# pagmerek/frave

Hardware: AMD Instinct MI355X
Metric: Mpixels/s encode (transform+quant) at 4096x4096 (higher is better)
Workload: dtype u8->i32

## Files before the change

### frave_amd/api.py

```python
import ctypes as C
import os
import subprocess

import numpy as np

_HERE = os.path.dirname(os.path.abspath(__file__))
_SO = os.environ.get("FRI_HIP_LIBRARY") or os.path.join(_HERE, "libfri_hip.so")
NONE = -(2 ** 31)

SYMBOLS = [
    "fri_hip_strerror", "fri_hip_version", "fri_hip_ctx_create", "fri_hip_ctx_destroy", "fri_hip_backend",
    "fri_hip_last_hip_error", "fri_hip_plan_create", "fri_hip_plan_destroy", "fri_hip_plan_num_cells",
    "fri_hip_plan_num_bfs_cells", "fri_hip_plan_num_interior_cells", "fri_hip_plan_coef_count", "fri_hip_plan_pixel_bytes",
    "fri_hip_plan_centers", "fri_hip_plan_valid_mask", "fri_hip_plan_num_some", "fri_hip_plan_neighbour_cells",
    "fri_hip_plan_neighbour_table", "fri_hip_plan_tiling", "fri_hip_plan_tile_table", "fri_hip_transform_quant", "fri_hip_transform_quant_dev",
    "fri_hip_transform_quant_batch_dev", "fri_hip_transform_quant_batch", "fri_hip_predict_histogram",
    "fri_hip_predict_histogram_dev", "fri_hip_fit_value_sums", "fri_hip_fit_value_sums_dev", "fri_hip_fit_width_sums",
    "fri_hip_fit_width_sums_dev", "fri_hip_inverse_transform", "fri_hip_inverse_transform_dev",
    "fri_hip_time_transform_quant_dev", "fri_hip_plan_read_trace", "fri_hip_plan_inverse_lists",
    "fri_hip_shard_size", "fri_hip_shard_image", "fri_hip_multi_create", "fri_hip_multi_destroy", "fri_hip_multi_num_devices",
    "fri_hip_multi_plan", "fri_hip_multi_transform_quant", "fri_hip_predict_histogram_batch_dev", "fri_hip_fit_value_sums_batch_dev",
    "fri_hip_fit_width_sums_batch_dev", "fri_hip_solve6", "fri_hip_fit_value_params", "fri_hip_fit_width_params", "fri_hip_encode_image",
    "fri_hip_encode_image_dev", "fri_hip_inverse_transform_batch_dev", "fri_hip_predict_image", "fri_hip_predict_image_dev",
    "fri_hip_fit_params_batch_dev", "fri_hip_encode_image_batch_dev", "fri_hip_fit_value_params_batch_dev", "fri_hip_fit_width_params_batch_dev",
    "fri_hip_plan_assume_forward_coefficients", "fri_hip_encode_image_batch", "fri_hip_multi_encode_image",
    "fri_hip_plan_set_stream_order", "fri_hip_symbol_stream_batch_dev", "fri_hip_encode_image_symbols", "fri_hip_encode_symbols_batch_dev",
    "fri_hip_plan_set_dequantiser", "fri_hip_plan_tune_forward", "fri_hip_time_transform_quant_streams_dev",
    "fri_hip_plan_set_colour_transform", "fri_hip_quality_matrix", "fri_hip_measure_distortion_dev", "fri_hip_search_quality",
    "fri_hip_search_quality_dev", "fri_hip_estimate_size_dev", "fri_hip_estimate_size", "fri_hip_search_quality_for_size",
    "fri_hip_search_quality_for_size_dev", "fri_hip_plan_predict_grid", "fri_hip_plan_pred_slots", "fri_hip_measure_ssim_dev", "fri_hip_measure_ssim", "fri_hip_search_quality_ssim",
    "fri_hip_search_quality_ssim_dev",
    "fri_hip_plan420_create", "fri_hip_plan420_destroy", "fri_hip_plan420_luma", "fri_hip_plan420_chroma", "fri_hip_split420_dev", "fri_hip_merge420_dev",
    "fri_hip_measure_distortion420_dev", "fri_hip_encode_image420_symbols", "fri_hip_decode_image420", "fri_hip_search_quality420", "fri_hip_search_quality420_dev",
    "fri_hip_search_quality_for_size420", "fri_hip_search_quality_for_size420_dev", "fri_hip_search_quality_ssim420", "fri_hip_search_quality_ssim420_dev",
    "fri_hip_plan_rgba_create", "fri_hip_plan_rgba_destroy", "fri_hip_plan_rgba_colour", "fri_hip_plan_rgba_alpha", "fri_hip_split_rgba_dev", "fri_hip_merge_rgba_dev",
    "fri_hip_encode_symbols_rgba_dev", "fri_hip_encode_image_rgba_symbols", "fri_hip_decode_image_rgba",
    "fri_hip_plan_owned_pixels", "fri_hip_tile_shape", "fri_hip_plan_tiled_create", "fri_hip_plan_tiled_destroy", "fri_hip_plan_tiled_tile", "fri_hip_plan_tiled_grid",
    "fri_hip_split_tiles_dev", "fri_hip_merge_tiles_dev", "fri_hip_encode_symbols_tiled_dev", "fri_hip_encode_image_tiled_symbols", "fri_hip_decode_image_tiled",
    "fri_hip_measure_distortion_tiled_dev", "fri_hip_estimate_size_tiled_dev", "fri_hip_estimate_size_tiled", "fri_hip_search_quality_tiled", "fri_hip_search_quality_tiled_dev",
    "fri_hip_search_quality_ssim_tiled", "fri_hip_search_quality_ssim_tiled_dev", "fri_hip_search_quality_for_size_tiled", "fri_hip_search_quality_for_size_tiled_dev",
    "fri_hip_rans_scratch_bytes", "fri_hip_rans_encode_planes_dev", "fri_hip_rans_time_planes_dev", "fri_hip_encode_image_tiled_coded",
    "fri_hip_plan_tiled_region", "fri_hip_merge_tiles_region_dev", "fri_hip_decode_region_tiled_dev", "fri_hip_decode_region_tiled",
    "fri_hip_plan_tiled_region_cover", "fri_hip_split_tiles_region_dev", "fri_hip_encode_symbols_region_tiled_dev", "fri_hip_encode_region_tiled_symbols",
    "fri_hip_tile_shape420", "fri_hip_plan_tiled420_create", "fri_hip_plan_tiled420_destroy", "fri_hip_plan_tiled420_luma", "fri_hip_plan_tiled420_chroma",
    "fri_hip_plan_tiled420_grid", "fri_hip_plan_tiled420_region", "fri_hip_plan_tiled420_buffer_tiles", "fri_hip_split_tiles420_dev", "fri_hip_merge_tiles420_dev",
    "fri_hip_merge_tiles420_region_dev", "fri_hip_encode_symbols_tiled420_dev", "fri_hip_encode_image_tiled420_symbols", "fri_hip_decode_image_tiled420",
    "fri_hip_decode_region_tiled420_dev", "fri_hip_decode_region_tiled420",
    "fri_hip_measure_distortion_tiled420_dev", "fri_hip_estimate_size_tiled420_dev", "fri_hip_estimate_size_tiled420", "fri_hip_search_quality_tiled420",
    "fri_hip_search_quality_tiled420_dev", "fri_hip_search_quality_ssim_tiled420", "fri_hip_search_quality_ssim_tiled420_dev", "fri_hip_search_quality_for_size_tiled420",
    "fri_hip_search_quality_for_size_tiled420_dev", "fri_hip_encode_image_tiled420_coded",
    "fri_hip_decode_scratch_bytes", "fri_hip_decode_planes_dev", "fri_hip_decode_time_planes_dev", "fri_hip_decode_image_tiled_coded", "fri_hip_decode_image_tiled420_coded",
    "fri_hip_plan_num_some_levels", "fri_hip_preview_size", "fri_hip_decode_planes_levels_dev", "fri_hip_preview_tiles_dev", "fri_hip_preview_image_tiled",
    "fri_hip_preview_image_tiled_coded",
    "fri_hip_plan_tiled_regions", "fri_hip_merge_tiles_regions_dev", "fri_hip_decode_regions_tiled_dev", "fri_hip_decode_regions_tiled",
    "fri_hip_decode_regions_tiled_coded",
    "fri_hip_plan_tiled_rgba_create", "fri_hip_plan_tiled_rgba_destroy", "fri_hip_plan_tiled_rgba_colour", "fri_hip_plan_tiled_rgba_alpha", "fri_hip_plan_tiled_rgba_grid",
    "fri_hip_plan_tiled_rgba_region", "fri_hip_plan_tiled_rgba_buffer_tiles", "fri_hip_split_tiles_rgba_dev", "fri_hip_merge_tiles_rgba_dev",
    "fri_hip_merge_tiles_rgba_region_dev", "fri_hip_encode_symbols_tiled_rgba_dev", "fri_hip_encode_image_tiled_rgba_symbols", "fri_hip_decode_image_tiled_rgba",
    "fri_hip_decode_region_tiled_rgba_dev", "fri_hip_decode_region_tiled_rgba",
]
DECODE_TRUNCATED, DECODE_BAD_MODEL, DECODE_BAD_SLOT = 1, 2, 4
RANS_EMPTY_OK = 1
RANS_TOO_SMALL, RANS_BAD_MODEL, RANS_ZERO_FREQ, RANS_BAD_BUCKET = 1, 2, 4, 8
TILED_ALLOW_HOLES = 1
ALPHA_KEEP, ALPHA_CLEAN = 0, 1
COLOUR_NONE, COLOUR_RCT, COLOUR_YCBCR = 0, 1, 3
DEQUANT_REFERENCE, DEQUANT_MULTIPLY, DEQUANT_MIDPOINT = 0, 1, 2


class FriHipError(RuntimeError):
    def __init__(self, code, where, detail=""):
        self.code = code
        msg = load_library().fri_hip_strerror(code).decode()
        super().__init__(f"{where}: {msg} ({code}){': ' + detail if detail else ''}")


def library_path():
    return _SO

# ... 59 lines not shown
    L.fri_hip_transform_quant_dev.argtypes = [vp, vp, vp, vp, vp]
    L.fri_hip_transform_quant_batch_dev.argtypes = [vp, u32, vp, sz, vp, vp, sz, vp]
    L.fri_hip_transform_quant_batch.argtypes = [vp, u32, vp, vp, vp]
    L.fri_hip_predict_histogram.argtypes = [vp, vp, u32, vp, vp, vp, vp, vp, vp]
    L.fri_hip_predict_histogram_dev.argtypes = [vp, vp, u32, vp, vp, vp, vp, vp, vp, vp]
    L.fri_hip_fit_value_sums.argtypes = [vp, vp, u32, vp]
    L.fri_hip_fit_value_sums_dev.argtypes = [vp, vp, u32, vp, vp]
    L.fri_hip_fit_width_sums.argtypes = [vp, vp, u32, vp, vp, vp, vp]
    L.fri_hip_fit_width_sums_dev.argtypes = [vp, vp, u32, vp, vp, vp, vp]
    L.fri_hip_inverse_transform.argtypes = [vp, vp, vp, vp]
    L.fri_hip_inverse_transform_dev.argtypes = [vp, vp, vp, vp, vp]
    L.fri_hip_plan_read_trace.argtypes = [vp, vp]
    L.fri_hip_plan_inverse_lists.argtypes = [vp, vp]
    L.fri_hip_plan_predict_grid.argtypes = [vp, vp]
    L.fri_hip_plan_pred_slots.argtypes = [vp, vp]
    L.fri_hip_time_transform_quant_dev.argtypes = [vp, u32, vp, sz, vp, vp, sz, u32, vp, C.POINTER(C.c_double)]
    L.fri_hip_time_transform_quant_streams_dev.argtypes = [vp, u32, vp, sz, vp, vp, sz, u32, u32, C.POINTER(C.c_double)]
    L.fri_hip_plan_tune_forward.argtypes = [vp, u32, C.c_char_p, sz]
    L.fri_hip_shard_size.restype, L.fri_hip_shard_size.argtypes = u32, [u32, u32, u32]
    L.fri_hip_shard_image.restype, L.fri_hip_shard_image.argtypes = u32, [u32, u32, u32]
    L.fri_hip_multi_create.argtypes = [vp, u32, u32, u32, u32, C.POINTER(vp)]
    L.fri_hip_multi_destroy.argtypes = [vp]
    L.fri_hip_multi_num_devices.restype, L.fri_hip_multi_num_devices.argtypes = u32, [vp]
    L.fri_hip_multi_plan.restype, L.fri_hip_multi_plan.argtypes = vp, [vp, u32]
    L.fri_hip_multi_transform_quant.argtypes = [vp, u32, vp, vp, vp]
    L.fri_hip_predict_histogram_batch_dev.argtypes = [vp, u32, vp, sz, vp, vp, vp, sz, vp, vp, vp]
    L.fri_hip_fit_value_sums_batch_dev.argtypes = [vp, u32, vp, sz, vp, vp]
    L.fri_hip_fit_width_sums_batch_dev.argtypes = [vp, u32, vp, sz, vp, vp, vp, vp]
    L.fri_hip_solve6.restype, L.fri_hip_solve6.argtypes = None, [vp, vp, vp]
    L.fri_hip_fit_value_params.restype, L.fri_hip_fit_value_params.argtypes = None, [vp, vp]
    L.fri_hip_fit_width_params.restype, L.fri_hip_fit_width_params.argtypes = None, [vp, vp, vp, vp]
    L.fri_hip_encode_image.argtypes = [vp, vp, vp, i32, vp, vp, vp, vp, vp, vp, vp]
    L.fri_hip_encode_image_dev.argtypes = [vp, vp, vp, i32, vp, vp, vp, vp, vp, vp, vp, vp]
    L.fri_hip_inverse_transform_batch_dev.argtypes = [vp, u32, vp, sz, vp, vp, sz, vp]
    L.fri_hip_predict_image.argtypes = [vp, vp, i32, vp, vp, vp, vp, vp, vp]
    L.fri_hip_predict_image_dev.argtypes = [vp, vp, i32, vp, vp, vp, vp, vp, vp, vp]
    L.fri_hip_fit_params_batch_dev.argtypes = [vp, u32, vp, sz, vp, vp, vp]
    L.fri_hip_plan_assume_forward_coefficients.argtypes = [vp, i32]
    L.fri_hip_plan_set_dequantiser.argtypes = [vp, i32]
    L.fri_hip_plan_set_colour_transform.argtypes = [vp, i32]
    L.fri_hip_quality_matrix.argtypes = [i32, vp]
    L.fri_hip_measure_distortion_dev.argtypes = [vp, vp, vp, vp, vp, vp]
    L.fri_hip_search_quality.argtypes = [vp, vp, C.c_double, vp, vp]
    L.fri_hip_search_quality_dev.argtypes = [vp, vp, C.c_double, vp, vp, vp]
    L.fri_hip_estimate_size_dev.argtypes = [vp, u32, vp, vp, vp, vp, vp]
    L.fri_hip_estimate_size.argtypes = [vp, vp, vp, vp]
    L.fri_hip_search_quality_for_size.argtypes = [vp, vp, C.c_uint64, vp, vp]
    L.fri_hip_search_quality_for_size_dev.argtypes = [vp, vp, C.c_uint64, vp, vp, vp]
    L.fri_hip_measure_ssim_dev.argtypes = [vp, u32, vp, vp, sz, vp, vp]
    L.fri_hip_measure_ssim.argtypes = [vp, vp, vp, vp]
    L.fri_hip_search_quality_ssim.argtypes = [vp, vp, C.c_double, vp, vp]
    L.fri_hip_search_quality_ssim_dev.argtypes = [vp, vp, C.c_double, vp, vp, vp]
    L.fri_hip_plan_set_stream_order.argtypes = [vp, vp, C.c_uint64]
    L.fri_hip_symbol_stream_batch_dev.argtypes = [vp, u32, vp, sz, vp, vp, sz, vp, sz, vp]
    L.fri_hip_encode_image_symbols.argtypes = [vp, vp, vp, i32, vp, vp, vp, vp, vp]
    L.fri_hip_encode_symbols_batch_dev.argtypes = [vp, u32, vp, sz, vp, i32, vp, vp, sz, vp, sz, vp, sz, vp, vp, vp, vp]
    L.fri_hip_encode_image_batch.argtypes = [vp, u32, vp, vp, i32, vp, vp, vp, vp, vp, vp]
    L.fri_hip_multi_encode_image.argtypes = [vp, u32, vp, vp, i32, vp, vp, vp, vp, vp, vp]
    L.fri_hip_fit_value_params_batch_dev.argtypes = [vp, u32, vp, vp, vp]
    L.fri_hip_fit_width_params_batch_dev.argtypes = [vp, u32, vp, vp, vp, vp]
    L.fri_hip_encode_image_batch_dev.argtypes = [vp, u32, vp, sz, vp, i32, vp, vp, sz, vp, vp, sz, vp, vp, vp, vp]
    L.fri_hip_plan420_create.argtypes = [vp, u32, u32, C.POINTER(vp)]
    L.fri_hip_plan420_destroy.argtypes = [vp]
    L.fri_hip_plan420_luma.restype, L.fri_hip_plan420_luma.argtypes = vp, [vp]
    L.fri_hip_plan420_chroma.restype, L.fri_hip_plan420_chroma.argtypes = vp, [vp]
    L.fri_hip_split420_dev.argtypes = [vp, vp, vp, vp, vp]
    L.fri_hip_merge420_dev.argtypes = [vp, vp, vp, vp, vp]
    L.fri_hip_measure_distortion420_dev.argtypes = [vp, vp, vp, vp, vp, vp]
    L.fri_hip_encode_image420_symbols.argtypes = [vp, vp, i32, vp, vp, vp, vp, vp]
    L.fri_hip_decode_image420.argtypes = [vp, vp, i32, vp]
    L.fri_hip_search_quality420.argtypes = [vp, vp, C.c_double, vp, vp]
    L.fri_hip_search_quality420_dev.argtypes = [vp, vp, C.c_double, vp, vp, vp]
    L.fri_hip_search_quality_for_size420.argtypes = [vp, vp, C.c_uint64, vp, vp]
    L.fri_hip_search_quality_for_size420_dev.argtypes = [vp, vp, C.c_uint64, vp, vp, vp]
    L.fri_hip_search_quality_ssim420.argtypes = [vp, vp, C.c_double, vp, vp]
    L.fri_hip_search_quality_ssim420_dev.argtypes = [vp, vp, C.c_double, vp, vp, vp]
    L.fri_hip_plan_rgba_create.argtypes = [vp, u32, u32, C.POINTER(vp)]
    L.fri_hip_plan_rgba_destroy.argtypes = [vp]
    L.fri_hip_plan_rgba_colour.restype, L.fri_hip_plan_rgba_colour.argtypes = vp, [vp]
    L.fri_hip_plan_rgba_alpha.restype, L.fri_hip_plan_rgba_alpha.argtypes = vp, [vp]
    L.fri_hip_split_rgba_dev.argtypes = [vp, vp, i32, vp, vp, vp]
    L.fri_hip_merge_rgba_dev.argtypes = [vp, vp, vp, vp, vp]
    L.fri_hip_encode_symbols_rgba_dev.argtypes = [vp, vp, i32, vp, i32, vp, vp, vp, vp, vp, vp]
    L.fri_hip_encode_image_rgba_symbols.argtypes = [vp, vp, i32, vp, vp, vp, vp, vp, vp]
    L.fri_hip_decode_image_rgba.argtypes = [vp, vp, vp, vp]
    L.fri_hip_plan_owned_pixels.restype, L.fri_hip_plan_owned_pixels.argtypes = C.c_uint64, [vp]
    L.fri_hip_tile_shape.argtypes = [u32, u32, u32, vp, vp]
    L.fri_hip_plan_tiled_create.argtypes = [vp, u32, u32, u32, u32, u32, u32, C.POINTER(vp)]
    L.fri_hip_plan_tiled_destroy.argtypes = [vp]
    L.fri_hip_plan_tiled_tile.restype, L.fri_hip_plan_tiled_tile.argtypes = vp, [vp]
    L.fri_hip_plan_tiled_grid.argtypes = [vp, vp]
    L.fri_hip_split_tiles_dev.argtypes = [vp, vp, vp, vp]
    L.fri_hip_merge_tiles_dev.argtypes = [vp, vp, vp, vp]
    L.fri_hip_encode_symbols_tiled_dev.argtypes = [vp, vp, vp, i32, vp, vp, vp, vp, vp, vp]
    L.fri_hip_encode_image_tiled_symbols.argtypes = [vp, vp, vp, vp, vp, vp, vp, vp]
    L.fri_hip_decode_image_tiled.argtypes = [vp, vp, vp, vp]
    L.fri_hip_plan_tiled_region.argtypes = [vp, u32, u32, u32, u32, vp]
    L.fri_hip_merge_tiles_region_dev.argtypes = [vp, vp, u32, u32, u32, u32, vp, vp]
    L.fri_hip_decode_region_tiled_dev.argtypes = [vp, vp, vp, u32, u32, u32, u32, vp, vp]
    L.fri_hip_decode_region_tiled.argtypes = [vp, vp, vp, u32, u32, u32, u32, vp]
    L.fri_hip_plan_tiled_regions.argtypes = [vp, u32, vp, vp, C.c_size_t, vp, vp, C.c_size_t]
    L.fri_hip_merge_tiles_regions_dev.argtypes = [vp, vp, u32, u32, vp, vp, vp]
    L.fri_hip_decode_regions_tiled_dev.argtypes = [vp, vp, vp, u32, vp, vp, vp]
    L.fri_hip_decode_regions_tiled.argtypes = [vp, vp, vp, u32, vp, vp]
    L.fri_hip_decode_regions_tiled_coded.argtypes = [vp, u32, vp, vp, C.c_size_t, vp, vp, vp, vp, vp, vp, vp, vp]
    L.fri_hip_plan_tiled_region_cover.argtypes = [vp, u32, u32, u32, u32, vp]
# ... 318 lines not shown


class Plan:

    def __init__(self, ctx, width, height, channels, _handle=None):
        self._h = None
        self.ctx = ctx
        self.width, self.height, self.channels = width, height, channels
        self.colour_transform = COLOUR_NONE
        self._owns = _handle is None
        if _handle is None:
            h = C.c_void_p()
            _check(load_library().fri_hip_plan_create(ctx._h if ctx else None, width, height, channels, C.byref(h)), "fri_hip_plan_create", ctx)
        else:
            h = C.c_void_p(_handle)
        self._h = h
        L = load_library()
        self.num_cells = L.fri_hip_plan_num_cells(h)
        self.num_bfs_cells = L.fri_hip_plan_num_bfs_cells(h)
        self.num_interior_cells = L.fri_hip_plan_num_interior_cells(h)
        self.coef_count = L.fri_hip_plan_coef_count(h)
        self.pixel_bytes = L.fri_hip_plan_pixel_bytes(h)
        self.num_some = L.fri_hip_plan_num_some(h)

    def close(self):
        if self._h:
            if self._owns:
                load_library().fri_hip_plan_destroy(self._h)
            self._h = None

    def __del__(self):
        try:
            self.close()
        except Exception:
            pass

    def num_some_levels(self, levels):
        out = C.c_uint64(0)
        _check(load_library().fri_hip_plan_num_some_levels(self._h, int(levels), C.byref(out)), "fri_hip_plan_num_some_levels", self.ctx)
        return int(out.value)

    def owned_pixels(self):
        return int(load_library().fri_hip_plan_owned_pixels(self._h))

    def set_stream_order(self, order=None):
        if order is None:
            from . import emit

            order = emit.stream_order(self.centers(), self.valid_mask())
        order = np.ascontiguousarray(order, np.uint32)
        _check(load_library().fri_hip_plan_set_stream_order(self._h, _p(order), order.size), "fri_hip_plan_set_stream_order", self.ctx)
        return order

    def symbol_stream_batch_dev(self, n_planes, d_coefs, coef_stride, d_bucket, d_prediction, out_stride, d_symbols, symbol_stride, stream=0):
        _check(load_library().fri_hip_symbol_stream_batch_dev(self._h, n_planes, d_coefs, coef_stride, d_bucket, d_prediction, out_stride, d_symbols, symbol_stride, stream),
               "fri_hip_symbol_stream_batch_dev", self.ctx)

    def encode_symbols_batch_dev(self, n_images, d_pixels, pixel_stride, qmatrix, fit, d_params, d_coefs, coef_stride, d_node_words, word_stride, d_symbols, symbol_stride,
                                 d_hist, d_oob, d_fit_range=0, stream=0):
        q = _q(qmatrix)
        _check(load_library().fri_hip_encode_symbols_batch_dev(self._h, n_images, d_pixels, pixel_stride, _p(q), 1 if fit else 0, d_params, d_coefs, coef_stride, d_node_words,
                                                               word_stride, d_symbols, symbol_stride, d_hist, d_oob, d_fit_range, stream), "fri_hip_encode_symbols_batch_dev", self.ctx)

    def set_dequantiser(self, multiply):
        mode = (1 if multiply else 0) if isinstance(multiply, bool) else int(multiply)
        _check(load_library().fri_hip_plan_set_dequantiser(self._h, mode), "fri_hip_plan_set_dequantiser")

    def measure_distortion_dev(self, d_coefs, d_reference_pixels, d_out, qmatrix=None, stream=0):
        q = _q(qmatrix)
        _check(load_library().fri_hip_measure_distortion_dev(self._h, d_coefs, _p(q), d_reference_pixels, d_out, stream), "fri_hip_measure_distortion_dev", self.ctx)

    def search_quality(self, pixels, target_db, stream=0):
        return _search(self, "fri_hip_search_quality", pixels, float(target_db), C.c_double, stream)

    def measure_ssim(self, a, b):
        pa, pb = np.ascontiguousarray(a, np.uint8), np.ascontiguousarray(b, np.uint8)
        assert pa.size == self.pixel_bytes and pb.size == self.pixel_bytes
        out = np.zeros(self.channels + 1, np.int64)
        _check(load_library().fri_hip_measure_ssim(self._h, _p(pa), _p(pb), _p(out)), "fri_hip_measure_ssim", self.ctx)
        return out

    def measure_ssim_dev(self, d_a, d_b, d_out, n_images=1, pixel_stride=0, stream=0):
        _check(load_library().fri_hip_measure_ssim_dev(self._h, n_images, d_a, d_b, pixel_stride, d_out, stream), "fri_hip_measure_ssim_dev", self.ctx)

    def search_quality_ssim(self, pixels, target, stream=0):
        return _search(self, "fri_hip_search_quality_ssim", pixels, float(target), C.c_double, stream)

    def estimate_size(self, hist, oob=None, stream=0, n_images=1, d_bytes=None, d_models=None):
        L = load_library()
        if isinstance(hist, int):
            assert d_bytes
            _check(L.fri_hip_estimate_size_dev(self._h, n_images, hist, oob or None, d_bytes, d_models or None, stream), "fri_hip_estimate_size_dev", self.ctx)
            return None
        h = np.ascontiguousarray(hist, np.uint32)
        assert h.size == self.channels * 10 * 1024
        o = None if oob is None else np.ascontiguousarray(oob, np.uint64)
        assert o is None or o.size == self.channels
        out = C.c_uint64(0)
        _check(L.fri_hip_estimate_size(self._h, _p(h), None if o is None else _p(o), C.byref(out)), "fri_hip_estimate_size", self.ctx)
        return out.value

    def search_quality_for_size(self, pixels, max_bytes, stream=0):
        return _search(self, "fri_hip_search_quality_for_size", pixels, int(max_bytes), C.c_uint64, stream)

    def set_colour_transform(self, mode):
        _check(load_library().fri_hip_plan_set_colour_transform(self._h, int(mode)), "fri_hip_plan_set_colour_transform")
# ... 875 lines not shown
```

### frave_amd/csrc/fri_hip.cpp

```cpp
#include "fri_hip_internal.hpp"

#include <atomic>
#include <cstdio>
#include <cstdlib>
#include <mutex>
#include <new>
#include <optional>
#include <thread>

#include "search_scaffold.hpp"
#include "solve6.hpp"

using namespace fri;
using namespace fri::host;

void PlanDelete::operator()(fri_hip_plan *p) const { delete p; }

struct fri_hip_multi {
    std::vector<fri_hip_ctx *> ctxs;
    std::vector<fri_hip_plan *> plans;
};

namespace {

template <typename T>
hipError_t upload(std::vector<DevMem<void>> &bufs, const std::vector<T> &v, const T *&out, size_t pad = 0) {
    auto &d = bufs.emplace_back();
    if (hipError_t e = hipMalloc(d.put(), std::max<size_t>(v.size() + pad, 1) * sizeof(T))) return e;
    if (pad)
        if (hipError_t e = hipMemset(static_cast<T *>(d.get()) + v.size(), 0, pad * sizeof(T))) return e;
    if (!v.empty())
        if (hipError_t e = hipMemcpy(d, v.data(), v.size() * sizeof(T), hipMemcpyHostToDevice)) return e;
    out = static_cast<const T *>(d.get());
    return hipSuccess;
}

std::vector<float> laplace_table() {
    static const float width[10] = {2.5f, 4.5f, 6.3f, 8.5f, 12.7f, 16.f, 20.f, 24.f, 28.f, 36.f};
    std::vector<float> t(10 * 1024);
    for (int b = 0; b < 10; b++)
        for (uint32_t j = 0; j < 1024; j++) {
            const float x = (float)((j & 1u) ? (int32_t)(j + 1) / -2 : (int32_t)(j / 2));
            t[b * 1024 + j] = std::exp(-std::fabs(x - 0.0f) / width[b]) / (2.0f * width[b]);
        }
    return t;
}

struct Knobs {
    int band_rows = 0, cells_per_tile = 0, cells_per_wg = 0, target_wgs = 0, tile_bytes = 0;
    int ranks = 0;
    std::optional<int> strided_shares;
    bool has_rank_weights = false;
    float rank_weight[4] = {0, 0, 0, 0};
    bool pins_forward = false;
    int batch_share_tiles = 0;
    std::optional<int> inv_shared, inv_strided_shares;
    int inv_band_rows = 0;
    int pred_blocks = 0, hist_blocks = 0, trace = 0, k3_scan = 0;
    int k1_ablate = 0, k2_ablate = 0, k3_ablate = 0, k4_ablate = 0;
    std::optional<int> k1_cached_stores, k1_batch_shares, k4_older_eighths;
};

Knobs read_knobs() {
    Knobs k;
    const char *on = std::getenv("FRI_HIP_TUNING");
    if (!on || on[0] != '1' || on[1] != 0) return k;
    auto env = [](const char *name) { return std::getenv(name); };
    auto pin = [&](const char *name) {
        const char *s = env(name);
        k.pins_forward |= s != nullptr;
        return s;
    };
    auto opt = [](const char *s) { return s ? std::optional<int>(std::atoi(s)) : std::nullopt; };
    auto num = [&](const char *s) { return opt(s).value_or(0); };
    k.band_rows = num(pin("FRI_HIP_BAND_ROWS")), k.cells_per_tile = num(pin("FRI_HIP_CELLS_PER_TILE")), k.cells_per_wg = num(pin("FRI_HIP_CELLS_PER_WG"));
    k.target_wgs = num(pin("FRI_HIP_TARGET_WGS")), k.tile_bytes = num(pin("FRI_HIP_TILE_BYTES")), k.ranks = std::min(num(pin("FRI_HIP_RANKS")), 4);
    k.strided_shares = opt(pin("FRI_HIP_STRIDED_SHARES"));
    if (const char *s = pin("FRI_HIP_RANK_WEIGHTS")) {
        float *w = k.rank_weight;
        k.has_rank_weights = std::sscanf(s, "%f,%f,%f,%f", &w[0], &w[1], &w[2], &w[3]) == 4;
    }
    k.batch_share_tiles = num(env("FRI_HIP_BATCH_SHARE_TILES"));
    k.inv_shared = opt(env("FRI_HIP_INV_SHARED")), k.inv_strided_shares = opt(env("FRI_HIP_INV_STRIDED_SHARES")), k.inv_band_rows = num(env("FRI_HIP_INV_BAND_ROWS"));
    k.pred_blocks = num(env("FRI_HIP_PRED_BLOCKS")), k.hist_blocks = num(env("FRI_HIP_HIST_BLOCKS")), k.trace = num(env("FRI_HIP_TRACE")), k.k3_scan = num(env("FRI_HIP_K3_SCAN"));
    k.k1_ablate = num(env("FRI_HIP_K1_ABLATE")), k.k2_ablate = num(env("FRI_HIP_K2_ABLATE")), k.k3_ablate = num(env("FRI_HIP_K3_ABLATE")), k.k4_ablate = num(env("FRI_HIP_K4_ABLATE"));
    k.k1_cached_stores = opt(env("FRI_HIP_K1_CACHED_STORES")), k.k1_batch_shares = opt(env("FRI_HIP_K1_BATCH_SHARES")), k.k4_older_eighths = opt(env("FRI_HIP_K4_OLDER_EIGHTHS"));
    return k;
}

int acquire_acc(fri_hip_plan *p, hipStream_t stream, uint32_t n_planes = 1) {
    fri_hip_ctx *c = p->ctx;
    HIP_TRY(c, hipSetDevice(c->device));
    if (p->acc_dirty) {
        HIP_TRY(c, hipDeviceSynchronize());
        for (auto &a : p->acc_slots) {
            if (a.pred_acc) HIP_TRY(c, hipMemset(a.pred_acc, 0, (size_t)a.planes * kPredAccWords * sizeof(uint32_t)));
            if (a.fit_acc) HIP_TRY(c, hipMemset(a.fit_acc, 0, (size_t)a.planes * kFitShards * kFitAccWords * sizeof(unsigned long long)));
        }
        HIP_TRY(c, hipDeviceSynchronize());
        p->acc_dirty = false;
    }
    int idx = -1;
    for (uint32_t i = 0; i < kPredAccRing && idx < 0; i++)
        if (p->acc_slots[i].used && p->acc_slots[i].stream == stream) idx = (int)i;
    for (uint32_t i = 0; i < kPredAccRing && idx < 0; i++)
        if (!p->acc_slots[i].used) {
            p->acc_slots[i].used = true;
            p->acc_slots[i].stream = stream;
            idx = (int)i;
        }
    if (idx < 0) {
        auto &v = p->acc_slots[p->acc_next];
        idx = (int)p->acc_next;
        p->acc_next = (p->acc_next + 1) % kPredAccRing;
        if (!v.handed_over) HIP_TRY(c, hipEventCreateWithFlags(v.handed_over.put(), hipEventDisableTiming));
        hipError_t e = hipEventRecord(v.handed_over, v.stream);
        if (e == hipSuccess) e = hipStreamWaitEvent(stream, v.handed_over, 0);
        if (e != hipSuccess) {
            (void)hipGetLastError();
            HIP_TRY(c, hipDeviceSynchronize());
        }
        v.stream = stream;
    }
    auto &a = p->acc_slots[idx];
    if (a.planes < n_planes) {
        const uint32_t planes = std::min<uint32_t>(65535u, std::max<uint32_t>({4u, n_planes, 2u * a.planes}));
        AccBufs n;
        const size_t pb = (size_t)planes * kPredAccWords * sizeof(uint32_t), fb = (size_t)planes * kFitShards * kFitAccWords * sizeof(unsigned long long);
        hipError_t e = hipMalloc((void **)n.pred_acc.put(), pb);
        if (e == hipSuccess) e = hipMalloc((void **)n.fit_acc.put(), fb);
        if (e == hipSuccess) e = hipMalloc((void **)n.sums_int.put(), (size_t)planes * 3 * 28 * sizeof(unsigned long long));
        if (e == hipSuccess) e = hipMalloc((void **)n.sums_dbl.put(), (size_t)planes * 18 * sizeof(double));
        if (e == hipSuccess) e = hipMalloc((void **)n.range.put(), (size_t)planes * sizeof(unsigned long long));
        if (e == hipSuccess) e = hipMalloc((void **)n.params.put(), (size_t)planes * sizeof(PredictParams));
        if (e == hipSuccess) e = hipMemsetAsync(n.pred_acc, 0, pb, stream);
        if (e == hipSuccess) e = hipMemsetAsync(n.fit_acc, 0, fb, stream);
        if (e != hipSuccess) return fail_hip(c, e, "accumulator allocation");
        std::swap(static_cast<AccBufs &>(a), n);
// ... 417 lines not shown
        build_inverse_lists(p->geo, kInvListsMaxBytes);
    }
    if (!ctx) {
        p->dev.n_pred_tiles = p->geo.n_pred_tiles;
        p->dev.pred_blocks = (uint32_t)std::max(k.pred_blocks, 0), p->dev.hist_blocks = (uint32_t)std::max(k.hist_blocks, 0);
        p->dev.k4_older_eighths = k.k4_older_eighths.value_or(0);
        *out = plan.release();
        return FRI_HIP_OK;
    }
    if (hipSetDevice(ctx->device) != hipSuccess) return FRI_HIP_ERR_HIP;
    const Geometry &g = p->geo, &gi = p->inv_geo();
    DevicePlan &d = p->dev;
    std::vector<uint16_t> tab(&st.nbr_table[0][0], &st.nbr_table[0][0] + kCell * 6);
    std::vector<uint32_t> gather_off((size_t)kCell * 4);
    std::vector<uint16_t> pair_pos(256), heap_of_pos(kCell);
    build_gather_tables(tab.data(), gather_off.data(), pair_pos.data(), heap_of_pos.data());
    std::vector<uint32_t> halo_list(1024);
    build_halo_list(tab.data(), pair_pos.data(), halo_list.data());
    build_lf_deltas(tab.data(), d.lf_delta);
    bool node0_gathered = false;
    for (int n = 2; n < kCell; n++)
        for (int i = 0; i < 6; i++) node0_gathered |= !(tab[(size_t)n * 6 + i] & 0x8000u) && (tab[(size_t)n * 6 + i] & 511u) == 0;
    if (halo_list[0] == 0xFFFFFFFFu || node0_gathered || pair_pos[0] != 0) {
        return FRI_HIP_ERR_INVALID_ARGUMENT;
    }
    auto &bufs = p->owned;
    hipError_t e;
    if ((e = upload_tiling(bufs, g, d, false)) || (e = upload(bufs, g.centers, d.centers)) || (e = upload(bufs, g.interior, d.interior)) || (e = upload(bufs, g.valid_mask, d.valid_mask)) ||
        (e = upload(bufs, g.nbr_cells, d.nbr_cells)) || (e = upload(bufs, g.pred_slots, d.pred_slots)) || (e = upload(bufs, tab, d.nbr_table)) ||
        (e = upload(bufs, gather_off, d.gather_off)) || (e = upload(bufs, pair_pos, d.pair_pos)) || (e = upload(bufs, heap_of_pos, d.heap_of_pos)) ||
        (e = upload(bufs, halo_list, d.halo_list)) || (e = upload(bufs, laplace_table(), p->laplace)))
        return fail_hip(ctx, e, "plan tables");
    if (!gi.inv_lists.empty()) {
        if ((e = upload(bufs, gi.inv_lists, d.inv_lists)) || (e = upload(bufs, gi.inv_quads, d.inv_quads, kInvListPad)) || (e = upload(bufs, gi.inv_dwords, d.inv_dwords, kInvListPad)) ||
            (e = upload(bufs, gi.inv_parts, d.inv_parts, kInvListPad)))
            return fail_hip(ctx, e, "inverse lists");
        d.inv_rect_bytes = gi.inv_rect_bytes;
    }
    d.F = (uint32_t)g.centers.size(), d.width = (int32_t)g.width, d.height = (int32_t)g.height, d.channels = (int32_t)g.channels, d.n_pred_tiles = g.n_pred_tiles;
    d.covers_image = g.n_valid_leaves == (uint64_t)g.width * g.height;
    d.inv_group = fwd.many_shares && g.wg_tiles.size() > 1 && (g.wg_tiles.size() - 1) % 1024 == 0 ? (int32_t)((g.wg_tiles.size() - 1) / 1024) : 1;
    d.inv_max_wg_tiles = d.inv_group > 1 ? 0 : d.max_wg_tiles, d.inv_max_wg_cells = d.inv_group > 1 ? 0 : d.max_wg_cells;
    for (size_t sh = 0; d.inv_group > 1 && sh + d.inv_group < g.wg_tiles.size(); sh += d.inv_group) {
        const Tile &first = g.tiles[g.wg_tiles[sh]], &last = g.tiles[g.wg_tiles[sh + d.inv_group] - 1];
        d.inv_max_wg_cells = std::max(d.inv_max_wg_cells, last.cell_begin + last.cell_count - first.cell_begin);
        d.inv_max_wg_tiles = std::max(d.inv_max_wg_tiles, g.wg_tiles[sh + d.inv_group] - g.wg_tiles[sh]);
    }
    d.pred_blocks = k.pred_blocks > 0 ? (uint32_t)k.pred_blocks : (uint32_t)ctx->cu_count;
    d.hist_blocks = k.hist_blocks > 0 ? (uint32_t)k.hist_blocks : 2u * (uint32_t)ctx->cu_count;
    d.k1_ablate = k.k1_ablate;
    if (k.k1_cached_stores) d.k1_cached_stores = *k.k1_cached_stores > 0 ? 1 : 0;
    if (k.k1_batch_shares) d.k1_batch_shares = *k.k1_batch_shares != 0;
    d.k2_ablate = k.k2_ablate;
    d.k3_ablate = k.k3_ablate;
    d.k3_scan = k.k3_scan > 0;
    d.k4_ablate = k.k4_ablate;
    if (k.k4_older_eighths) d.k4_older_eighths = *k.k4_older_eighths;
    if (hipMalloc(bufs.emplace_back().put(), (size_t)d.pred_blocks * kPredJunkWaves * kPredJunkBytes) != hipSuccess) return FRI_HIP_ERR_HIP;
    d.junk = static_cast<uint8_t *>(bufs.back().get());
    if (k.trace > 0) {
        const size_t bytes = (size_t)std::max<size_t>(d.n_wg, p->own_inverse_tiling ? gi.wg_tiles.size() : 0) * 16 * sizeof(unsigned long long);
        auto &t = bufs.emplace_back();
        if (hipMalloc(t.put(), bytes) != hipSuccess || hipMemset(t, 0, bytes) != hipSuccess) return FRI_HIP_ERR_HIP;
        d.trace = static_cast<unsigned long long *>(t.get());
    }
    if (hipEventCreate(p->ev_begin.put()) != hipSuccess || hipEventCreate(p->ev_end.put()) != hipSuccess) return FRI_HIP_ERR_HIP;
    p->dev_inv = d;
    if (p->own_inverse_tiling && (e = upload_tiling(bufs, gi, p->dev_inv, true))) return fail_hip(ctx, e, "inverse tiling");
    p->fwd_tunable = p->own_inverse_tiling && !fwd.many_shares && !d.trace && !k.pins_forward;
    if (p->fwd_tunable) adopt_cached_forward_tiling(p);
    *out = plan.release();
    return FRI_HIP_OK;
}

int fri_hip_plan_destroy(fri_hip_plan *p) {
    if (p && p->ctx) (void)hipSetDevice(p->ctx->device);
    delete p;
    return FRI_HIP_OK;
}

uint32_t fri_hip_plan_num_cells(const fri_hip_plan *p) { return p ? (uint32_t)p->geo.centers.size() : 0; }
uint32_t fri_hip_plan_num_bfs_cells(const fri_hip_plan *p) { return p ? p->geo.n_bfs_cells : 0; }
uint32_t fri_hip_plan_num_interior_cells(const fri_hip_plan *p) { return p ? p->geo.n_interior : 0; }
size_t fri_hip_plan_coef_count(const fri_hip_plan *p) { return p ? (size_t)p->geo.channels * p->geo.centers.size() * kCell : 0; }
size_t fri_hip_plan_pixel_bytes(const fri_hip_plan *p) { return p ? (size_t)p->geo.width * p->geo.height * p->geo.channels : 0; }
uint64_t fri_hip_plan_num_some(const fri_hip_plan *p) { return p ? p->geo.n_some : 0; }
int fri_hip_plan_num_some_levels(const fri_hip_plan *p, uint32_t levels, uint64_t *out) {
    if (!p || !out || levels > (uint32_t)kDepth) return FRI_HIP_ERR_INVALID_ARGUMENT;
    *out = num_some_levels(p->geo, levels);
    return FRI_HIP_OK;
}
int fri_hip_preview_size(uint32_t width, uint32_t height, uint32_t shift, uint32_t out[2]) {
    if (!width || !height || shift > 4 || !out) return FRI_HIP_ERR_INVALID_ARGUMENT;
    const uint32_t S = 1u << shift;
    out[0] = (uint32_t)(((uint64_t)width + S - 1) / S), out[1] = (uint32_t)(((uint64_t)height + S - 1) / S);
    return FRI_HIP_OK;
}
uint64_t fri_hip_plan_owned_pixels(const fri_hip_plan *p) { return p ? p->geo.n_valid_leaves : 0; }

int fri_hip_plan_assume_forward_coefficients(fri_hip_plan *p, int on) {
    if (!p) return FRI_HIP_ERR_INVALID_ARGUMENT;
    p->assume_forward = on != 0;
    return FRI_HIP_OK;
}

int fri_hip_plan_set_dequantiser(fri_hip_plan *p, int mode) {
// ... 379 lines not shown
}

void fri_hip_fit_width_params(const int64_t wtw[3][21], const double wtr[3][6], const uint64_t rows[3], float width_params[3][6]) {
    Solve6Work w;
    for (int g = 0; g < 3; g++) fit_width_group(reinterpret_cast<const long long *>(wtw[g]), wtr[g], rows[g], width_params[g], w);
}

class Coefs16Lease {
  public:
    Coefs16Lease(fri_hip_plan *p, hipStream_t s, size_t planes) : p_(p), s_(s) { rc = take(planes); }
    ~Coefs16Lease() {
        if (rc) return;
        p_->coefs16_stream = s_, p_->coefs16_used = true;
        if (hipEventRecord(p_->ev_coefs16, s_) != hipSuccess) {
            (void)hipGetLastError();
            (void)hipDeviceSynchronize();
            p_->coefs16_used = false;
        }
    }
    Coefs16Lease(const Coefs16Lease &) = delete;
    Coefs16Lease &operator=(const Coefs16Lease &) = delete;
    int rc;

  private:
    int take(size_t planes) {
        fri_hip_ctx *c = p_->ctx;
        if (int r = grow(c, p_->coefs16, planes * p_->geo.centers.size() * kCell)) return r;
        if (!p_->ev_coefs16) HIP_TRY(c, hipEventCreateWithFlags(p_->ev_coefs16.put(), hipEventDisableTiming));
        if (p_->coefs16_used && p_->coefs16_stream != s_) HIP_TRY(c, hipStreamWaitEvent(s_, p_->ev_coefs16, 0));
        return FRI_HIP_OK;
    }
    fri_hip_plan *p_;
    hipStream_t s_;
};

static int fit_chain(fri_hip_plan *p, const PredBatch &b, unsigned long long *d_range, hipStream_t s, float *host_params = nullptr, unsigned long long *host_range = nullptr,
                     int trust = kPredAnyInt32) {
    if (!b.params) return FRI_HIP_ERR_INVALID_ARGUMENT;
    const int slot = acquire_acc(p, s, b.n_planes);
    if (slot < 0) return slot;
    auto &k = p->acc_slots[slot];
    float *params = const_cast<float *>(reinterpret_cast<const float *>(b.params));
    const uint64_t F = p->geo.centers.size();
    const unsigned long long rows[3] = {F * 256, F * 128, F * 128};
    unsigned long long *range = d_range ? d_range : k.range;
    FitSolve solve;
    solve.params = params, solve.host_params = host_params, solve.host_range = host_range;
    for (int g = 0; g < 3; g++) solve.rows[g] = rows[g];
    if (int rc = fit_launch(p, 0, b, (int64_t *)k.sums_int.get(), nullptr, range, s, &solve, trust)) return rc;
    solve.host_range = nullptr;
    return fit_launch(p, 1, b, (int64_t *)k.sums_int.get(), k.sums_dbl, nullptr, s, &solve, trust);
}

static int predict_image_dev(fri_hip_plan *p, const int32_t *d_coefs, int fit, float *value_params, float *width_params, uint8_t *d_bucket, int32_t *d_prediction,
                             uint32_t *d_hist, uint64_t *d_oob, int trust, hipStream_t s, uint16_t *d_words = nullptr, const int16_t *d_coefs16 = nullptr,
                             uint16_t *d_streams = nullptr) {
    fri_hip_ctx *c = p->ctx;
    const uint32_t C = p->geo.channels;
    const size_t plane = p->geo.centers.size() * kCell;
    PredBatch b;
    b.n_planes = C;
    b.coefs = d_coefs;
    b.coefs16 = d_coefs16;
    b.coef_stride = plane;
    b.out_stride = plane;
    b.words = d_words;
    if (d_streams) b.words = d_streams, b.out_stride = p->geo.n_some, b.stream_pos = p->d_stream_pos;
    if (!fit) {
        for (uint32_t ch = 0; ch < C; ch++) {
            std::memcpy(b.pp[ch].value, value_params + ch * 18, sizeof(b.pp[ch].value));
            std::memcpy(b.pp[ch].width, width_params + ch * 18, sizeof(b.pp[ch].width));
        }
        return predict_launch(p, b, d_bucket, d_prediction, d_hist, d_oob, trust, s);
    }
    const int slot = acquire_acc(p, s, C);
    if (slot < 0) return slot;
    auto &k = p->acc_slots[slot];
    constexpr size_t kFitBytes = 3 * sizeof(PredictParams) + 3 * sizeof(unsigned long long);
    if (!p->d_h_fit) {
        HIP_TRY(c, hipHostMalloc(p->h_fit.put(), kFitBytes, hipHostMallocMapped | hipHostMallocCoherent));
        std::memset(p->h_fit, 0, kFitBytes);
        HIP_TRY(c, hipHostGetDevicePointer(&p->d_h_fit, p->h_fit, 0));
    }
    if (!p->ev_fit) HIP_TRY(c, hipEventCreateWithFlags(p->ev_fit.put(), hipEventDisableTiming));
    b.params = reinterpret_cast<const PredictParams *>(k.params.get());
    char *const h = static_cast<char *>(p->h_fit.get()), *const dh = static_cast<char *>(p->d_h_fit);
    if (int rc = fit_chain(p, b, k.range, s, reinterpret_cast<float *>(dh), reinterpret_cast<unsigned long long *>(dh + 3 * sizeof(PredictParams)), trust)) return rc;
    HIP_TRY(c, hipEventRecord(p->ev_fit, s));
    const int rc_scan = predict_launch(p, b, d_bucket, d_prediction, d_hist, d_oob, trust, s);
    if (int rc = wait_event_polling(c, p->ev_fit)) return rc;
    std::atomic_thread_fence(std::memory_order_acquire);
    const unsigned long long *h_range = reinterpret_cast<const unsigned long long *>(h + 3 * sizeof(PredictParams));
    const PredictParams *h_params = reinterpret_cast<const PredictParams *>(h);
    for (uint32_t ch = 0; ch < C; ch++) {
        std::memcpy(value_params + ch * 18, h_params[ch].value, sizeof(h_params[ch].value));
        std::memcpy(width_params + ch * 18, h_params[ch].width, sizeof(h_params[ch].width));
    }
    for (uint32_t ch = 0; ch < C; ch++)
        if (h_range[ch]) return FRI_HIP_ERR_OUT_OF_RANGE;
    return rc_scan;
}

int fri_hip_encode_image_dev(fri_hip_plan *p, const uint8_t *d_pixels, const int32_t qmatrix[32], int fit, float *value_params, float *width_params, int32_t *d_coefs,
                             uint8_t *d_bucket, int32_t *d_prediction, uint32_t *d_hist, uint64_t *d_n_out_of_alphabet, void *stream) {
    if (int rc = need_device(p)) return rc;
    if (!d_pixels || !value_params || !width_params || !d_coefs || !d_hist || !d_n_out_of_alphabet) return FRI_HIP_ERR_INVALID_ARGUMENT;
    QMatrix q;
    if (int rc = check_q(qmatrix, q)) return rc;
    if (int rc = refuse_capture(p, (hipStream_t)stream)) return rc;
    HIP_TRY(p->ctx, hipSetDevice(p->ctx->device));
    HIP_TRY(p->ctx, launch_fwd_transform_quant(p->dev, 1, d_pixels, 0, d_coefs, 0, q, (hipStream_t)stream, chain_wants_cached_coefficients(p, 1, fit)));
    return predict_image_dev(p, d_coefs, fit, value_params, width_params, d_bucket, d_prediction, d_hist, d_n_out_of_alphabet, kPredForwardOutput, (hipStream_t)stream);
}

int fri_hip_encode_image_batch_dev(fri_hip_plan *p, uint32_t n_images, const uint8_t *d_pixels, size_t pixel_stride, const int32_t qmatrix[32], int fit, float *d_params,
                                   int32_t *d_coefs, size_t coef_stride, uint8_t *d_bucket, int32_t *d_prediction, size_t out_stride, uint32_t *d_hist,
                                   uint64_t *d_n_out_of_alphabet, uint64_t *d_fit_out_of_range, void *stream) {
    if (int rc = need_device(p)) return rc;
    const uint32_t C = p->geo.channels;
    const size_t plane = p->geo.centers.size() * kCell, image = (size_t)C * plane;
    if (!d_pixels || !d_params || !d_coefs || !d_hist || !d_n_out_of_alphabet || !n_images || (uint64_t)n_images * C > 65535u) return FRI_HIP_ERR_INVALID_ARGUMENT;
    if (n_images > 1 && (pixel_stride < fri_hip_plan_pixel_bytes(p) || coef_stride < image || ((d_bucket || d_prediction) && out_stride < image))) return FRI_HIP_ERR_INVALID_ARGUMENT;
    if (C > 1 && n_images > 1 && (coef_stride != image || ((d_bucket || d_prediction) && out_stride != image))) return FRI_HIP_ERR_INVALID_ARGUMENT;
    QMatrix q;
    if (int rc = check_q(qmatrix, q)) return rc;
    hipStream_t s = (hipStream_t)stream;
    if (int rc = refuse_capture(p, s)) return rc;
    HIP_TRY(p->ctx, hipSetDevice(p->ctx->device));
    HIP_TRY(p->ctx, launch_fwd_transform_quant(p->dev, n_images, d_pixels, pixel_stride, d_coefs, coef_stride, q, s, chain_wants_cached_coefficients(p, n_images, fit)));
    PredBatch b;
    b.n_planes = n_images * C;
    b.coefs = d_coefs;
    b.coef_stride = C > 1 ? plane : coef_stride;
    b.out_stride = C > 1 ? plane : out_stride;
    b.params = reinterpret_cast<const PredictParams *>(d_params);
    if (fit)
        if (int rc = fit_chain(p, b, (unsigned long long *)d_fit_out_of_range, s, nullptr, nullptr, kPredForwardOutput)) return rc;
    return predict_launch(p, b, d_bucket, d_prediction, d_hist, d_n_out_of_alphabet, kPredForwardOutput, s);
}

int fri_hip_encode_symbols_batch_dev(fri_hip_plan *p, uint32_t n_images, const uint8_t *d_pixels, size_t pixel_stride, const int32_t qmatrix[32], int fit, float *d_params,
                                     int32_t *d_coefs, size_t coef_stride, uint16_t *d_node_words, size_t word_stride, uint16_t *d_symbols, size_t symbol_stride,
                                     uint32_t *d_hist, uint64_t *d_n_out_of_alphabet, uint64_t *d_fit_out_of_range, void *stream) {
    if (int rc = need_device(p)) return rc;
    const uint32_t C = p->geo.channels;
    const size_t plane = p->geo.centers.size() * kCell, image = (size_t)C * plane, n = p->geo.n_some;
    if (!d_pixels || !d_params || !d_symbols || !d_hist || !d_n_out_of_alphabet || !n_images || (uint64_t)n_images * C > 65535u || !p->d_stream_order)
        return FRI_HIP_ERR_INVALID_ARGUMENT;
    const bool compact = d_coefs == nullptr;
    const bool direct = d_node_words == nullptr;
    if (direct && !compact) return FRI_HIP_ERR_INVALID_ARGUMENT;
    if (compact) coef_stride = image;
    if (direct) word_stride = image;
    if (n_images > 1 && (pixel_stride < fri_hip_plan_pixel_bytes(p) || coef_stride < image || word_stride < image || symbol_stride < (size_t)C * n)) return FRI_HIP_ERR_INVALID_ARGUMENT;
    if (C > 1 && n_images > 1 && (coef_stride != image || word_stride != image || symbol_stride != (size_t)C * n)) return FRI_HIP_ERR_INVALID_ARGUMENT;
    QMatrix q;
    if (int rc = check_q(qmatrix, q)) return rc;
    hipStream_t s = (hipStream_t)stream;
    if (int rc = refuse_capture(p, s)) return rc;
    HIP_TRY(p->ctx, hipSetDevice(p->ctx->device));
    std::optional<Coefs16Lease> lease;
    if (compact && lease.emplace(p, s, (size_t)n_images * C).rc) return lease->rc;
    HIP_TRY(p->ctx, launch_fwd_transform_quant(p->dev, n_images, d_pixels, pixel_stride, d_coefs, coef_stride, q, s, chain_wants_cached_coefficients(p, n_images, fit),
                                               compact ? p->coefs16.get() : nullptr));
    PredBatch b;
    b.n_planes = n_images * C;
    b.coefs = d_coefs;
    b.coefs16 = compact ? p->coefs16.get() : nullptr;
    b.coef_stride = C > 1 || compact ? plane : coef_stride;
    b.out_stride = C > 1 ? plane : word_stride;
    b.params = reinterpret_cast<const PredictParams *>(d_params);
    b.words = d_node_words;
    if (direct) b.words = d_symbols, b.out_stride = C > 1 ? n : symbol_stride, b.stream_pos = p->d_stream_pos;
    if (fit)
        if (int rc = fit_chain(p, b, (unsigned long long *)d_fit_out_of_range, s, nullptr, nullptr, kPredForwardOutput)) return rc;
    if (int rc = predict_launch(p, b, nullptr, nullptr, d_hist, d_n_out_of_alphabet, kPredForwardOutput, s)) return rc;
    if (!direct) HIP_TRY(p->ctx, launch_symbol_gather(p->d_stream_order, n, b.n_planes, d_node_words, b.out_stride, d_symbols, C > 1 ? n : symbol_stride, s));
    return FRI_HIP_OK;
}

int fri_hip_fit_value_params_batch_dev(fri_hip_plan *p, uint32_t n_planes, const int64_t *d_gram, float *d_params, void *stream) {
    if (int rc = need_device(p)) return rc;
    if (!d_gram || !d_params || !n_planes || n_planes > 65535u) return FRI_HIP_ERR_INVALID_ARGUMENT;
    HIP_TRY(p->ctx, hipSetDevice(p->ctx->device));
    HIP_TRY(p->ctx, launch_fit_solve(0, n_planes, reinterpret_cast<const unsigned long long *>(d_gram), nullptr, nullptr, d_params, (hipStream_t)stream));
    return FRI_HIP_OK;
}

int fri_hip_fit_width_params_batch_dev(fri_hip_plan *p, uint32_t n_planes, const int64_t *d_wtw, const double *d_wtr, float *d_params, void *stream) {
    if (int rc = need_device(p)) return rc;
    if (!d_wtw || !d_wtr || !d_params || !n_planes || n_planes > 65535u) return FRI_HIP_ERR_INVALID_ARGUMENT;
    HIP_TRY(p->ctx, hipSetDevice(p->ctx->device));
    const uint64_t F = p->geo.centers.size();
    const unsigned long long rows[3] = {F * 256, F * 128, F * 128};
    HIP_TRY(p->ctx, launch_fit_solve(1, n_planes, reinterpret_cast<const unsigned long long *>(d_wtw), d_wtr, rows, d_params, (hipStream_t)stream));
    return FRI_HIP_OK;
}

int fri_hip_fit_params_batch_dev(fri_hip_plan *p, uint32_t n_planes, const int32_t *d_coefs, size_t coef_stride, float *d_params, uint64_t *d_fit_out_of_range, void *stream) {
    if (int rc = need_device(p)) return rc;
    if (!d_coefs || !d_params || !n_planes || n_planes > 65535u || (n_planes > 1 && coef_stride < p->geo.centers.size() * kCell)) return FRI_HIP_ERR_INVALID_ARGUMENT;
    HIP_TRY(p->ctx, hipSetDevice(p->ctx->device));
    PredBatch b;
    b.n_planes = n_planes;
    b.coefs = d_coefs;
    b.coef_stride = coef_stride;
    b.params = reinterpret_cast<const PredictParams *>(d_params);
    return fit_chain(p, b, (unsigned long long *)d_fit_out_of_range, (hipStream_t)stream);
}

int fri_hip_predict_image_dev(fri_hip_plan *p, const int32_t *d_coefs, int fit, float *value_params, float *width_params, uint8_t *d_bucket, int32_t *d_prediction,
                              uint32_t *d_hist, uint64_t *d_n_out_of_alphabet, void *stream) {
    if (int rc = need_device(p)) return rc;
    if (!d_coefs || !value_params || !width_params || !d_hist || !d_n_out_of_alphabet) return FRI_HIP_ERR_INVALID_ARGUMENT;
    if (int rc = refuse_capture(p, (hipStream_t)stream)) return rc;
    HIP_TRY(p->ctx, hipSetDevice(p->ctx->device));
    return predict_image_dev(p, d_coefs, fit, value_params, width_params, d_bucket, d_prediction, d_hist, d_n_out_of_alphabet, kPredAnyInt32, (hipStream_t)stream);
}

int fri_hip_predict_image(fri_hip_plan *p, const int32_t *coefs, int fit, float *value_params, float *width_params, uint8_t *bucket, int32_t *prediction, uint32_t *hist,
                          uint64_t *n_out_of_alphabet) {
    if (int rc = need_device(p)) return rc;
    if (!coefs || !value_params || !width_params || !hist || !n_out_of_alphabet) return FRI_HIP_ERR_INVALID_ARGUMENT;
    fri_hip_ctx *c = p->ctx;
    HIP_TRY(c, hipSetDevice(c->device));
    const size_t C = p->geo.channels, plane = p->geo.centers.size() * kCell;
// ... 55 lines not shown
        HIP_TRY(c, hipStreamSynchronize(s.stream));
        std::memcpy(coefs[i], s.h_coefs, n * sizeof(int32_t));
        if (bucket && bucket[i]) std::memcpy(bucket[i], s.h_bucket, n);
        if (prediction && prediction[i]) std::memcpy(prediction[i], s.h_prediction, n * sizeof(int32_t));
        std::memcpy(hist[i], s.h_hist, C * 10 * 1024 * sizeof(uint32_t));
        std::memcpy(n_out_of_alphabet[i], s.h_oob, C * sizeof(uint64_t));
        if (fit) std::memcpy(params[i], s.h_params, C * sizeof(PredictParams));
        for (size_t ch = 0; ch < C; ch++)
            if (fit && s.h_oob[C + ch]) first_error = first_error ? first_error : FRI_HIP_ERR_OUT_OF_RANGE;
        return FRI_HIP_OK;
    };
    for (Slot &s : p->slots) s.pending = -1;
    for (uint32_t i = 0; i < n_images; i++) {
        if (!pixels[i] || !params[i] || !coefs[i] || !hist[i] || !n_out_of_alphabet[i]) return FRI_HIP_ERR_INVALID_ARGUMENT;
        Slot &s = p->slots[i % kBatchSlots];
        if (int rc = drain(s)) return rc;
        std::memcpy(s.h_pixels, pixels[i], pb);
        HIP_TRY(c, hipMemcpyAsync(s.d_pixels, s.h_pixels, pb, hipMemcpyHostToDevice, s.stream));
        if (!fit) {
            std::memcpy(s.h_params, params[i], C * sizeof(PredictParams));
            HIP_TRY(c, hipMemcpyAsync(s.d_params, s.h_params, C * sizeof(PredictParams), hipMemcpyHostToDevice, s.stream));
        }
        if (int rc = fri_hip_encode_image_batch_dev(p, 1, s.d_pixels, 0, qmatrix, fit, s.d_params, s.d_coefs, 0, bucket && bucket[i] ? s.d_bucket : nullptr,
                                                    prediction && prediction[i] ? s.d_prediction : nullptr, 0, s.d_hist, (uint64_t *)s.d_oob.get(), (uint64_t *)(s.d_oob + C), s.stream))
            return rc;
        HIP_TRY(c, hipMemcpyAsync(s.h_coefs, s.d_coefs, n * sizeof(int32_t), hipMemcpyDeviceToHost, s.stream));
        if (bucket && bucket[i]) HIP_TRY(c, hipMemcpyAsync(s.h_bucket, s.d_bucket, n, hipMemcpyDeviceToHost, s.stream));
        if (prediction && prediction[i]) HIP_TRY(c, hipMemcpyAsync(s.h_prediction, s.d_prediction, n * sizeof(int32_t), hipMemcpyDeviceToHost, s.stream));
        HIP_TRY(c, hipMemcpyAsync(s.h_hist, s.d_hist, C * 10 * 1024 * sizeof(uint32_t), hipMemcpyDeviceToHost, s.stream));
        HIP_TRY(c, hipMemcpyAsync(s.h_oob, s.d_oob, 2 * C * sizeof(unsigned long long), hipMemcpyDeviceToHost, s.stream));
        if (fit) HIP_TRY(c, hipMemcpyAsync(s.h_params, s.d_params, C * sizeof(PredictParams), hipMemcpyDeviceToHost, s.stream));
        s.pending = (int)i;
    }
    for (Slot &s : p->slots)
        if (int rc = drain(s)) return rc;
    return first_error;
}

int fri_hip_multi_encode_image(fri_hip_multi *m, uint32_t n_images, const uint8_t *const *pixels, const int32_t qmatrix[32], int fit, float *const *params,
                               int32_t *const *coefs, uint8_t *const *bucket, int32_t *const *prediction, uint32_t *const *hist, uint64_t *const *n_out_of_alphabet) {
    if (!m || !pixels || !params || !coefs || !hist || !n_out_of_alphabet || !qmatrix) return FRI_HIP_ERR_INVALID_ARGUMENT;
    return run_shards(m, n_images, [&](fri_hip_plan *p, const std::vector<uint32_t> &images) {
        const auto in = pick(pixels, images);
        const auto par = pick(params, images);
        const auto co = pick(coefs, images), pr = pick(prediction, images);
        const auto bu = pick(bucket, images);
        const auto hi = pick(hist, images);
        const auto oo = pick(n_out_of_alphabet, images);
        return fri_hip_encode_image_batch(p, (uint32_t)images.size(), in.data(), qmatrix, fit, par.data(), co.data(), bucket ? bu.data() : nullptr,
                                          prediction ? pr.data() : nullptr, hi.data(), oo.data());
    });
}

int fri_hip_plan_set_stream_order(fri_hip_plan *p, const uint32_t *order, uint64_t n) {
    if (int rc = need_device(p)) return rc;
    if (!order || n != p->geo.n_some) return FRI_HIP_ERR_INVALID_ARGUMENT;
    const size_t F = p->geo.centers.size();
    std::vector<uint8_t> seen(F * kCell, 0);
    for (uint64_t i = 0; i < n; i++) {
        const uint32_t e = order[i], cell = e >> 9, heap = e & 511u;
        if (cell >= F || !((p->geo.valid_mask[(size_t)cell * 16 + (heap >> 5)] >> (heap & 31)) & 1u) || seen[e]) return FRI_HIP_ERR_INVALID_ARGUMENT;
        seen[e] = 1;
    }
    fri_hip_ctx *c = p->ctx;
    HIP_TRY(c, hipSetDevice(c->device));
    std::vector<uint32_t> pos(F * kCell, 0xFFFFFFFFu);
    for (uint64_t i = 0; i < n; i++) pos[order[i]] = (uint32_t)i;
    DevMem<uint32_t> d_order, d_pos;
    HIP_TRY(c, hipMalloc((void **)d_order.put(), (n ? n : 1) * sizeof(uint32_t)));
    HIP_TRY(c, hipMemcpy(d_order, order, n * sizeof(uint32_t), hipMemcpyHostToDevice));
    HIP_TRY(c, hipMalloc((void **)d_pos.put(), pos.size() * sizeof(uint32_t)));
    HIP_TRY(c, hipMemcpy(d_pos, pos.data(), pos.size() * sizeof(uint32_t), hipMemcpyHostToDevice));
    p->d_stream_order = std::move(d_order), p->d_stream_pos = std::move(d_pos);
    return FRI_HIP_OK;
}

int fri_hip_symbol_stream_batch_dev(fri_hip_plan *p, uint32_t n_planes, const int32_t *d_coefs, size_t coef_stride, const uint8_t *d_bucket, const int32_t *d_prediction,
                                    size_t out_stride, uint16_t *d_symbols, size_t symbol_stride, void *stream) {
    if (int rc = need_device(p)) return rc;
    if (!p->d_stream_order) return FRI_HIP_ERR_INVALID_ARGUMENT;
    const size_t plane = p->geo.centers.size() * kCell;
    if (!d_coefs || !d_bucket || !d_prediction || !d_symbols || !n_planes || n_planes > 65535u) return FRI_HIP_ERR_INVALID_ARGUMENT;
    if (n_planes > 1 && (coef_stride < plane || out_stride < plane || symbol_stride < p->geo.n_some)) return FRI_HIP_ERR_INVALID_ARGUMENT;
    HIP_TRY(p->ctx, hipSetDevice(p->ctx->device));
    HIP_TRY(p->ctx, launch_symbol_stream(p->d_stream_order, p->geo.n_some, n_planes, d_coefs, coef_stride, d_bucket, d_prediction, out_stride, d_symbols, symbol_stride,
                                         (hipStream_t)stream));
    return FRI_HIP_OK;
}

int fri_hip_encode_image_symbols(fri_hip_plan *p, const uint8_t *pixels, const int32_t qmatrix[32], int fit, float *value_params, float *width_params, uint16_t *symbols,
                                 uint32_t *hist, uint64_t *n_out_of_alphabet) {
    if (int rc = need_device(p)) return rc;
    if (!pixels || !value_params || !width_params || !symbols || !hist || !n_out_of_alphabet || !p->d_stream_order) return FRI_HIP_ERR_INVALID_ARGUMENT;
    fri_hip_ctx *c = p->ctx;
    HIP_TRY(c, hipSetDevice(c->device));
    const size_t C = p->geo.channels, n = p->geo.n_some;
    auto &st = p->staging;
    int rc;
    if ((rc = grow(c, st.pixels, fri_hip_plan_pixel_bytes(p))) || (rc = grow(c, st.hist, C * 10 * 1024)) || (rc = grow(c, st.oob, C)) ||
        (rc = grow(c, st.symbols, std::max<size_t>(C * n, 1))))
        return rc;
    QMatrix q;
    if ((rc = check_q(qmatrix, q))) return rc;
    HIP_TRY(c, hipMemcpy(st.pixels, pixels, fri_hip_plan_pixel_bytes(p), hipMemcpyHostToDevice));
    {
        Coefs16Lease lease(p, nullptr, C);
        if (lease.rc) return lease.rc;
        HIP_TRY(c, launch_fwd_transform_quant(p->dev, 1, st.pixels, 0, nullptr, 0, q, nullptr, false, p->coefs16));
        if ((rc = predict_image_dev(p, nullptr, fit, value_params, width_params, nullptr, nullptr, st.hist, (uint64_t *)st.oob.get(), kPredForwardOutput, nullptr, nullptr,
                                    p->coefs16, st.symbols)))
            return rc;
    }
    HIP_TRY(c, hipMemcpy(symbols, st.symbols, C * n * sizeof(uint16_t), hipMemcpyDeviceToHost));
    HIP_TRY(c, hipMemcpy(hist, st.hist, C * 10 * 1024 * sizeof(uint32_t), hipMemcpyDeviceToHost));
    HIP_TRY(c, hipMemcpy(n_out_of_alphabet, st.oob, C * sizeof(uint64_t), hipMemcpyDeviceToHost));
    return FRI_HIP_OK;
}

int fri_hip_inverse_transform_batch_dev(fri_hip_plan *p, uint32_t n_images, const int32_t *d_coefs, size_t coef_stride, const int32_t qmatrix[32], uint8_t *d_pixels,
                                        size_t pixel_stride, void *stream) {
    if (int rc = need_device(p)) return rc;
    if (!d_coefs || !d_pixels || !n_images || n_images > 65535u) return FRI_HIP_ERR_INVALID_ARGUMENT;
    if (n_images > 1 && (pixel_stride < fri_hip_plan_pixel_bytes(p) || coef_stride < fri_hip_plan_coef_count(p))) return FRI_HIP_ERR_INVALID_ARGUMENT;
    QMatrix q;
    if (int rc = check_q(qmatrix, q)) return rc;
    HIP_TRY(p->ctx, launch_inverse_transform(p->dev_inv, n_images, d_coefs, coef_stride, q, d_pixels, pixel_stride, (hipStream_t)stream));
// ... 350 lines not shown
```

### frave_amd/csrc/fri_hip_internal.hpp

```cpp
#pragma once
#include "fri_hip.h"

#include <hip/hip_runtime_api.h>

#include <algorithm>
#include <cmath>
#include <cstring>
#include <memory>
#include <string>
#include <utility>
#include <vector>

#include "geometry.hpp"
#include "kernels.hpp"

struct fri_hip_ctx {
    int device = -1;
    std::string arch;
    int cu_count = 256;
    std::string last_error;
    float *rans_laplace = nullptr;
};

namespace fri::host {
// ... 58 lines not shown
    DevMem<int32_t> d_coefs;
    int pending = -1;
    HostMem<uint8_t> h_bucket;
    DevMem<uint8_t> d_bucket;
    HostMem<int32_t> h_prediction;
    DevMem<int32_t> d_prediction;
    HostMem<uint32_t> h_hist;
    DevMem<uint32_t> d_hist;
    HostMem<unsigned long long> h_oob;
    DevMem<unsigned long long> d_oob;
    HostMem<float> h_params;
    DevMem<float> d_params;
};

struct PlanDelete {
    void operator()(fri_hip_plan *p) const;
};

struct AccBufs {
    DevMem<uint32_t> pred_acc;
    DevMem<unsigned long long> fit_acc;
    DevMem<unsigned long long> sums_int;
    DevMem<double> sums_dbl;
    DevMem<unsigned long long> range;
    DevMem<float> params;
};

struct Plan {
    fri_hip_ctx *ctx = nullptr;
    Geometry geo;
    DevicePlan dev;
    Geometry geo_inv;
    bool own_inverse_tiling = false;
    DevicePlan dev_inv;
    const Geometry &inv_geo() const { return own_inverse_tiling ? geo_inv : geo; }
    std::vector<DevMem<void>> owned;
    Staging staging;
    Slot slots[kBatchSlots];
    bool slots_ready = false;
    struct AccSlot : AccBufs {
        hipStream_t stream = nullptr;
        bool used = false;
        Event handed_over;
        uint32_t pred_serial = 0;
        uint32_t planes = 0;
    } acc_slots[kPredAccRing];
    std::vector<AccBufs> retired_acc;
    HostMem<void> h_fit;
    void *d_h_fit = nullptr;
    Event ev_fit;
    const float *laplace = nullptr;
    bool assume_forward = false;
    DevMem<uint32_t> d_stream_order;
    DevMem<uint32_t> d_stream_pos;
    Grown<int16_t> coefs16;
    Event ev_coefs16;
    hipStream_t coefs16_stream = nullptr;
    bool coefs16_used = false;
    uint32_t acc_next = 0;
    bool acc_dirty = false;
    Event ev_begin, ev_end;
    TilingParams fwd_tp;
    bool fwd_tunable = false;
    std::string fwd_tiling_note = "default";
};

}

struct fri_hip_plan : fri::host::Plan {};

namespace fri::host {

inline int fail_hip(fri_hip_ctx *ctx, hipError_t e, const char *what) {
    if (ctx) {
        ctx->last_error = std::string(what) + ": " + hipGetErrorString(e);
    }
    return e == hipErrorOutOfMemory ? FRI_HIP_ERR_OUT_OF_MEMORY : FRI_HIP_ERR_HIP;
}

#define HIP_TRY(ctx, expr)                                 \
    do {                                                   \
        hipError_t e_ = (expr);                            \
        if (e_ != hipSuccess) return fail_hip(ctx, e_, #expr); \
    } while (0)

template <typename T>
int grow(fri_hip_ctx *c, Grown<T> &b, size_t n) {
    if (b.n >= n) return FRI_HIP_OK;
    b.n = 0;
    HIP_TRY(c, hipMalloc((void **)b.put(), n * sizeof(T)));
    b.n = n;
    return FRI_HIP_OK;
}

inline constexpr RateLayout kRateLayout = {16 + 2, (2 + 36 * 4) + (2 + 8) + 2 + 60, 2 + 4 + 8};

inline int check_q(const int32_t q[32], QMatrix &out) {
    if (!q) return FRI_HIP_ERR_INVALID_ARGUMENT;
    for (int i = 0; i < 32; i++) out.q[i] = q[i];
    for (int i = 0; i <= 9; i++)
        if (q[i] == 0) return FRI_HIP_ERR_DIVIDE_BY_ZERO;
    return FRI_HIP_OK;
}

template <typename AnyPlan>
int need_device(const AnyPlan *p) {
    if (!p) return FRI_HIP_ERR_INVALID_ARGUMENT;
// ... 95 lines not shown
```

### frave_amd/csrc/k2_predict.hip

```cpp
#include "gather_common.hpp"

#include <algorithm>
#include <vector>

namespace fri {
namespace {

__device__ __forceinline__ uint32_t f32_as_u32(float x) {
    uint32_t r;
    asm("v_cvt_u32_f32 %0, %1" : "=v"(r) : "v"(x));
    return r;
}
__device__ __forceinline__ int f32_as_i32(float x) {
    int r;
    asm("v_cvt_i32_f32 %0, %1" : "=v"(r) : "v"(x));
    return r;
}
__host__ __device__ constexpr uint32_t bucket_of(uint32_t w) {
    return w < 3 ? 0 : w < 5 ? 1 : w < 6 ? 2 : w < 8 ? 3 : w < 12 ? 4 : w < 16 ? 5 : w < 20 ? 6 : w < 25 ? 7 : w < 30 ? 8 : 9;
}
__host__ __device__ constexpr uint32_t bucket_plane(int bit) {
    uint32_t m = 0;
    for (uint32_t w = 0; w < 32; w++) m |= ((bucket_of(w) >> bit) & 1u) << w;
    return m;
}
__device__ __forceinline__ uint32_t bucket_of_rt(uint32_t width_u32) {
    const uint32_t w = min(width_u32, 31u);
    constexpr uint32_t P0 = bucket_plane(0), P1 = bucket_plane(1), P2 = bucket_plane(2), P3 = bucket_plane(3);
    return __builtin_amdgcn_ubfe(P0, w, 1) | (__builtin_amdgcn_ubfe(P1, w, 1) << 1) | (__builtin_amdgcn_ubfe(P2, w, 1) << 2) |
           (__builtin_amdgcn_ubfe(P3, w, 1) << 3);
}
__device__ __forceinline__ uint32_t assign_bucket(float width) { return bucket_of_rt(f32_as_u32(width)); }
__device__ __forceinline__ uint32_t pack_signed(int k) { return ((uint32_t)k << 1) ^ (uint32_t)(k >> 31); }

constexpr int kLfNever = 127;
struct PredArgs {
    const int32_t *coefs;
    const int32_t *pred_slots;
    const uint16_t *nbr_table;
    const uint32_t *pred_off;
    const uint16_t *pair_pos;
    const uint16_t *heap_of_pos;
    const uint32_t *halo_list;
    uint32_t *inexact;
    size_t coef_stride, out_stride;
    const PredictParams *params;
    int32_t ablate;
    const uint8_t *interior;
    const uint32_t *valid_mask;
    uint8_t *bucket;
    int32_t *prediction;
    uint32_t *hist;
    unsigned long long *n_oob;
    uint8_t *junk;
    unsigned long long *trace;
    uint32_t *acc;
    int8_t lf_delta[8];
    uint32_t serial;
    uint32_t n_tiles;
    uint16_t *words;
    const uint32_t *stream_pos;
    int32_t trusted;
    PredictParams pp;
    PredictParams pp3[3];
};

constexpr int kAccZeroFlag = 0, kAccTicket = 12, kAccInexact = 14;
constexpr uint32_t kPredZeroBlocks = 10;
static_assert(kAccInexact + 2 == (int)kPredAccWords && kAccZeroFlag + (int)kPredZeroBlocks <= kAccTicket, "accumulator layout");
__device__ __forceinline__ void pred_clear_issue(const PredArgs &a, int tid, int n_threads) {
    const uint32_t nz = min(gridDim.x, kPredZeroBlocks);
    if (blockIdx.x >= nz) return;
    for (uint32_t c = blockIdx.x; c < 10u; c += nz)
        for (uint32_t j = (uint32_t)tid; j < 1024u; j += (uint32_t)n_threads) (void)__hip_atomic_exchange(a.hist + c * 1024u + j, 0u, __ATOMIC_RELAXED, __HIP_MEMORY_SCOPE_AGENT);
    if (blockIdx.x == 0 && tid == 0) (void)__hip_atomic_exchange(a.n_oob, 0ull, __ATOMIC_RELAXED, __HIP_MEMORY_SCOPE_AGENT);
}
__device__ __forceinline__ void pred_clear_publish(const PredArgs &a, int tid) {
    if (blockIdx.x < min(gridDim.x, kPredZeroBlocks) && tid == 0)
        (void)__hip_atomic_exchange(a.acc + kAccZeroFlag + blockIdx.x, a.serial, __ATOMIC_RELAXED, __HIP_MEMORY_SCOPE_AGENT);
}
__device__ __forceinline__ uint32_t pred_clear_poll(const PredArgs &a, int lane) {
    return (uint32_t)lane < min(gridDim.x, kPredZeroBlocks) ? __hip_atomic_load(a.acc + kAccZeroFlag + lane, __ATOMIC_RELAXED, __HIP_MEMORY_SCOPE_AGENT) : a.serial;
}
template <bool CHECK>
__device__ __forceinline__ void pred_hand_over(const PredArgs &a, const uint32_t *s_hist, uint32_t *s_flag, int tid, int n_threads, uint32_t early_poll) {
    if (!__all(early_poll == a.serial)) {
        const int lane = tid & 63;
        while (!__all(pred_clear_poll(a, lane) == a.serial)) __builtin_amdgcn_s_sleep(2);
    }
    asm volatile("" ::: "memory");
    for (int i = tid; i < kHistBins; i += n_threads) {
        const uint32_t c = s_hist[i];
        if (c) (void)__hip_atomic_fetch_add(a.hist + i, c, __ATOMIC_RELAXED, __HIP_MEMORY_SCOPE_AGENT);
    }
    if (tid == 0 && s_hist[kHistBins]) (void)__hip_atomic_fetch_add(a.n_oob, (unsigned long long)s_hist[kHistBins], __ATOMIC_RELAXED, __HIP_MEMORY_SCOPE_AGENT);
    if (!CHECK) return;
    wait_for_own_memory_ops_then_barrier();
    if (tid == 0) *s_flag = __hip_atomic_fetch_add(a.acc + kAccTicket, 1u, __ATOMIC_RELAXED, __HIP_MEMORY_SCOPE_AGENT) == gridDim.x - 1 ? 1u : 0u;
    __syncthreads();
    if (*s_flag == 0) return;
    const bool inexact = __hip_atomic_load(a.inexact, __ATOMIC_RELAXED, __HIP_MEMORY_SCOPE_AGENT) != 0;
    if (inexact) {
        for (int i = tid; i < kHistBins; i += n_threads) (void)__hip_atomic_exchange(a.hist + i, 0u, __ATOMIC_RELAXED, __HIP_MEMORY_SCOPE_AGENT);
        if (tid == 0) {
            (void)__hip_atomic_exchange(a.n_oob, a.trusted ? ~0ull : 0ull, __ATOMIC_RELAXED, __HIP_MEMORY_SCOPE_AGENT);
            if (a.trusted) __hip_atomic_store(a.inexact, 0u, __ATOMIC_RELAXED, __HIP_MEMORY_SCOPE_AGENT);
        }
    }
    if (tid == 0) __hip_atomic_store(a.acc + kAccTicket, 0u, __ATOMIC_RELAXED, __HIP_MEMORY_SCOPE_AGENT);
}

struct P3Lds {
    uint32_t hist[kHistBins + 4];
    uint8_t cells[2][kP3ImageBytes];
    int32_t ring[3][kPredSlots];
    uint16_t bkt[32];
    uint32_t masks[2][kPredSlots][16];
// ... 167 lines not shown
        for (int j = 0; j < 4; j++) {
            const bool lf = ROLE == 0 && j < 2 && lane == 0;
            if (!lf && !(ablate & 4)) atomicAdd(reinterpret_cast<uint32_t *>(reinterpret_cast<uint8_t *>(s_hist) + bin[j]), 1u);
        }
        leave(pred, b12);
    } else {
        int pm[4];
        uint32_t bm[4];
#pragma unroll
        for (int j = 0; j < 4; j++) {
            const bool some = (some4 >> j) & 1u;
            if (some && !(ablate & 4)) atomicAdd(reinterpret_cast<uint32_t *>(reinterpret_cast<uint8_t *>(s_hist) + bin[j]), 1u);
            pm[j] = some ? pred[j] : 0;
            bm[j] = some ? b12[j] : 0u;
        }
        leave(pm, bm);
    }
}

struct P3LfItem {
    int raw;
    int nb[3];
    int node;
};
__device__ __forceinline__ void p3_lf_hop_a(const PredArgs &a, uint32_t tile, bool active, int tid, P3LfItem &it) {
    const int c = (tid & 31) >> 1;
    it.node = tid & 1;
    const int slot = (1 + c / kPredBlock) * kPredSide + 1 + (c % kPredBlock);
    const int32_t *row = a.pred_slots + (size_t)(active ? tile : 0) * kPredSlots;
    it.raw = row[slot];
#pragma unroll
    for (int k = 0; k < 3; k++) {
        const int d0 = a.lf_delta[k], d1 = a.lf_delta[3 + k];
        const int delta = it.node ? d1 : d0;
        const int r = row[slot + (delta == kLfNever ? 0 : delta)];
        it.nb[k] = delta == kLfNever ? -1 : r;
    }
    if (!active) it.raw = -1;
}
struct P3LfValues {
    int v[3], value;
    uint32_t mask0;
};
template <bool C16 = false>
__device__ __forceinline__ void p3_lf_hop_b(const PredArgs &a, const int32_t *plane, const P3LfItem &it, P3LfValues &x) {
    const uint32_t n = (uint32_t)it.node;
    auto at = [&](int cell) -> int { return C16 ? (int)(reinterpret_cast<const int16_t *>(plane) + (size_t)cell * kCell)[n] : (plane + (size_t)cell * kCell)[n]; };
#pragma unroll
    for (int k = 0; k < 3; k++) x.v[k] = at(max(pred_slot_cell(it.nb[k]), 0));
    const int cell = max(pred_slot_cell(it.raw), 0);
    x.value = at(cell);
    x.mask0 = a.valid_mask[(size_t)cell * 16];
}
template <bool WORDS, bool STREAM = false>
__device__ __forceinline__ void p3_lf_finish(const PredArgs &a, uint32_t *s_hist, const P3LfItem &it, const P3LfValues &x) {
    const int cell = pred_slot_cell(it.raw);
    if (cell < 0) return;
    int v[3];
#pragma unroll
    for (int k = 0; k < 3; k++) v[k] = it.nb[k] < 0 || x.v[k] == kNone ? 0 : x.v[k];
    uint32_t b12;
    int prediction;
    p3_lf(v[0], v[1], v[2], b12, prediction);
    const bool some = pred_slot_interior(it.raw) || ((x.mask0 >> it.node) & 1u);
    const uint32_t sym = pack_signed(sub_w(x.value, prediction));
    const uint32_t counter = sym < 1024u ? (b12 >> 2) + sym : (uint32_t)kHistBins;
    if (some) atomicAdd(&s_hist[counter], 1u);
    if (WORDS && STREAM) {
        if (some) a.words[a.stream_pos[(size_t)cell * kCell + it.node]] = (uint16_t)counter;
        return;
    }
    if (WORDS) {
        a.words[(size_t)cell * kCell + it.node] = (uint16_t)counter;
        return;
    }
    if (a.prediction) a.prediction[(size_t)cell * kCell + it.node] = some ? prediction : 0;
    if (a.bucket) a.bucket[(size_t)cell * kCell + it.node] = (uint8_t)(some ? b12 >> 12 : 0u);
}

struct ExactArgs {
    const int32_t *coefs;
    const uint16_t *nbr_table;
    const int32_t *nbr_cells;
    const uint8_t *interior;
    const uint32_t *valid_mask;
    uint8_t *bucket;
    int32_t *prediction;
    uint32_t *hist;
    unsigned long long *n_oob;
    uint32_t *acc;
    uint32_t F;
    PredictParams pp;
    size_t coef_stride, out_stride;
    const PredictParams *params;
    PredictParams pp3[3];
};
__global__ void __launch_bounds__(kCell) exact_predict_kernel(const ExactArgs a0) {
    ExactArgs a = a0;
    {
        const uint32_t plane = blockIdx.y;
        a.coefs += plane * a0.coef_stride;
        if (a.bucket) a.bucket += plane * a0.out_stride;
        if (a.prediction) a.prediction += plane * a0.out_stride;
        a.hist += (size_t)plane * kHistBins;
        a.n_oob += plane;
        a.acc += (size_t)plane * kPredAccWords;
    }
    PredictParams pp;
    if (a0.params)
        pp = a0.params[blockIdx.y];
    else if (blockIdx.y == 0)
        pp = a0.pp3[0];
    else if (blockIdx.y == 1)
        pp = a0.pp3[1];
    else
        pp = a0.pp3[2];
    uint32_t *const inexact = a.acc + kAccInexact;
    __shared__ uint32_t s_go;
    if (threadIdx.x == 0) s_go = __hip_atomic_load(inexact, __ATOMIC_RELAXED, __HIP_MEMORY_SCOPE_AGENT);
    __syncthreads();
    if (s_go == 0) return;
    const int p = threadIdx.x;
// ... 57 lines not shown
    }
}

__device__ __forceinline__ int p3_some_or_zero(int v) { return v == kNone ? 0 : v; }
template <bool CHECK>
__device__ __forceinline__ float p3_pack2(int x, int y, uint32_t &d) {
    const float f0 = (float)x, f1 = (float)y;
    d = __builtin_amdgcn_perm(__builtin_bit_cast(uint32_t, f1), __builtin_bit_cast(uint32_t, f0), 0x07060302u);
    return CHECK ? __builtin_fmaxf(__builtin_fabsf(f0), __builtin_fabsf(f1)) : 0.f;
}
template <bool CHECK>
__device__ __forceinline__ float p3_commit4(int raw, i32x4 v, uint8_t *dst, uint32_t pos0, uint32_t pos1) {
    if (!pred_slot_interior(raw)) {
        if (raw < 0)
            v = i32x4{0, 0, 0, 0};
        else
            v = i32x4{p3_some_or_zero(v.x), p3_some_or_zero(v.y), p3_some_or_zero(v.z), p3_some_or_zero(v.w)};
    }
    uint32_t d0, d1;
    const float m = __builtin_fmaxf(p3_pack2<CHECK>(v.x, v.y, d0), p3_pack2<CHECK>(v.z, v.w, d1));
    *reinterpret_cast<uint32_t *>(dst + pos0) = d0;
    *reinterpret_cast<uint32_t *>(dst + pos1) = d1;
    return m;
}
__device__ __forceinline__ void p3_check(float m, int lane, uint32_t *inexact) {
    if (__builtin_expect(__any(m > 256.0f), 0) && lane == 0) __hip_atomic_store(inexact, 1u, __ATOMIC_RELAXED, __HIP_MEMORY_SCOPE_AGENT);
}
struct P3Halo {
    int raw, v;
};
template <bool C16 = false>
__device__ __forceinline__ void p3_issue_halo(const int32_t *plane, const int32_t *slots, uint32_t ring_off, uint32_t heap_off, P3Halo &h) {
    h.raw = *reinterpret_cast<const int32_t *>(reinterpret_cast<const uint8_t *>(slots) + ring_off);
    const uint32_t cell = (uint32_t)max(h.raw, 0) & (uint32_t)(kPredSlotInterior - 1);
    if (C16)
        h.v = *reinterpret_cast<const int16_t *>(reinterpret_cast<const uint8_t *>(plane) + ((cell << 10) + (heap_off >> 1)));
    else
        h.v = *reinterpret_cast<const int32_t *>(reinterpret_cast<const uint8_t *>(plane) + ((cell << 11) + heap_off));
}
template <bool CHECK>
__device__ __forceinline__ float p3_commit_halo(const P3Halo &h, uint8_t *image, uint32_t lds_off) {
    const int v = (h.raw < 0 || h.v == kNone) ? 0 : h.v;
    const float f = (float)v;
    *reinterpret_cast<uint16_t *>(image + lds_off) = (uint16_t)(__builtin_bit_cast(uint32_t, f) >> 16);
    return CHECK ? __builtin_fabsf(f) : 0.f;
}

struct P3Lane {
    uint32_t addr[4][6];
    uint32_t opos[2];
    uint32_t halo_ring;
    uint32_t halo_heap;
    uint32_t halo_lds;
};

template <int ROLE, bool C16 = false>
__device__ __forceinline__ i32x4 p3_load_own(const int32_t *plane, size_t cell, uint32_t lane) {
    if (C16) {
        const int16_t *cell_base = reinterpret_cast<const int16_t *>(plane) + cell * kCell;
        if (ROLE) {
            const i32x2 d = reinterpret_cast<const i32x2 *>(cell_base + 256)[lane];
            return i32x4{d.x, d.y, 0, 0};
        }
        return i32x4{reinterpret_cast<const int32_t *>(cell_base)[lane], reinterpret_cast<const int32_t *>(cell_base + 128)[lane], 0, 0};
    }
    const int32_t *cell_base = plane + cell * kCell;
    if (ROLE) return reinterpret_cast<const i32x4 *>(cell_base + 256)[lane];
    const i32x2 a = reinterpret_cast<const i32x2 *>(cell_base)[lane], b = reinterpret_cast<const i32x2 *>(cell_base + 128)[lane];
    return i32x4{a.x, a.y, b.x, b.y};
}
template <bool C16>
__device__ __forceinline__ void p3_unpack_own(i32x4 &v) {
    if (C16) v = i32x4{(int)(short)v.x, v.x >> 16, (int)(short)v.y, v.y >> 16};
}
template <int ROLE>
__device__ __forceinline__ u32x4 p3_load_pos(const uint32_t *stream_pos, size_t cell, uint32_t lane) {
    const uint32_t *base = stream_pos + cell * kCell;
    if (ROLE) return reinterpret_cast<const u32x4 *>(base + 256)[lane];
    const i32x2 a = reinterpret_cast<const i32x2 *>(base)[lane], b = reinterpret_cast<const i32x2 *>(base + 128)[lane];
    return u32x4{(uint32_t)a.x, (uint32_t)a.y, (uint32_t)b.x, (uint32_t)b.y};
}

template <int IMG, int ROLE, bool CHECK, bool WORDS, bool C16 = false, bool STREAM = false>
__device__ __forceinline__ void p3_tile(const PredArgs &a, const int32_t *plane, P3Lds &lds, int it, bool more, uint32_t next2_tile, int tid, int lane, int wave, int slot_a,
                                        const P3Lane &L, float (&ga)[6], float (&gb)[6], const i32x4 (&own_cur)[2], i32x4 (&own_nxt)[2], const u32x4 (&pos_cur)[2],
                                        u32x4 (&pos_nxt)[2]) {
    uint32_t *s_hist = lds.hist;
    const uint16_t *s_bkt = lds.bkt;
    const int32_t *cur_slots = lds.ring[it % 3], *nxt_slots = lds.ring[(it + 1) % 3];
    const int32_t slot_pre = a.pred_slots[(size_t)next2_tile * kPredSlots + tid % kPredSlots];
    uint32_t st_own_mask[2];
    P3Halo st_halo;
    int raw_own[2] = {-1, -1};
    if (ablate_flags(a.ablate) & 2) more = false;
    if (more) {
#pragma unroll
        for (int c = 0; c < 2; c++) {
            raw_own[c] = __builtin_amdgcn_readfirstlane(nxt_slots[slot_a + c]);
            const int cell = max(pred_slot_cell(raw_own[c]), 0);
            own_nxt[c] = p3_load_own<ROLE, C16>(plane, (size_t)cell, (uint32_t)lane);
            if (STREAM) pos_nxt[c] = p3_load_pos<ROLE>(a.stream_pos, (size_t)cell, (uint32_t)lane);
            if (ROLE == 1) st_own_mask[c] = (a.valid_mask + (size_t)cell * 16)[(uint32_t)lane & 15u];
        }
        p3_issue_halo<C16>(plane, nxt_slots, L.halo_ring, L.halo_heap, st_halo);
    }

#pragma unroll
    for (int c = 0; c < 2; c++) {
        const int raw = (ablate_flags(a.ablate) & 1) ? -1 : __builtin_amdgcn_readfirstlane(cur_slots[slot_a + c]);
        const int cell = pred_slot_cell(raw);
        const bool has = cell >= 0, interior = pred_slot_interior(raw);
        const size_t junk = ((size_t)blockIdx.x * kP3Waves + wave) * kPredJunkBytes;
        uint8_t *bd = has && a.bucket ? a.bucket + (size_t)cell * kCell : a.junk + junk;
        int32_t *pd = has && a.prediction ? a.prediction + (size_t)cell * kCell : reinterpret_cast<int32_t *>(a.junk + junk + 512);
        uint16_t *wd = WORDS && STREAM ? a.words : WORDS && has ? a.words + (size_t)cell * kCell : reinterpret_cast<uint16_t *>(a.junk + junk + 512);
        const uint32_t pos4[4] = {pos_cur[c].x, pos_cur[c].y, pos_cur[c].z, pos_cur[c].w};
        uint32_t some4 = 0;
        if (!interior && has) {
            const uint32_t *m = lds.masks[IMG][slot_a + c];
            if (ROLE) {
                some4 = (m[8 + (lane >> 3)] >> (4 * (lane & 7))) & 15u;
            } else {
                some4 = ((m[lane >> 4] >> (2 * (lane & 15))) & 3u) | (((m[4 + (lane >> 4)] >> (2 * (lane & 15))) & 3u) << 2);
                if (lane == 0) some4 &= ~3u;
            }
        }
        const int own4[4] = {own_cur[c].x, own_cur[c].y, own_cur[c].z, own_cur[c].w};
        if (WORDS && (ablate_flags(a.ablate) & 1)) {
            if (ROLE) {
                __builtin_nontemporal_store(i32x2{0, 0}, reinterpret_cast<i32x2 *>(wd + 256) + lane);
            } else {
                __builtin_nontemporal_store(0u, reinterpret_cast<uint32_t *>(wd) + lane);
                __builtin_nontemporal_store(0u, reinterpret_cast<uint32_t *>(wd + 128) + lane);
            }
        } else if (ablate_flags(a.ablate) & 1) {
            if (ROLE) {
                __builtin_nontemporal_store(i32x4{0, 0, 0, 0}, reinterpret_cast<i32x4 *>(pd + 256) + lane);
                __builtin_nontemporal_store(0u, reinterpret_cast<uint32_t *>(bd + 256) + lane);
            } else {
                __builtin_nontemporal_store(i32x2{0, 0}, reinterpret_cast<i32x2 *>(pd) + lane);
                __builtin_nontemporal_store((uint16_t)0, reinterpret_cast<uint16_t *>(bd) + lane);
                __builtin_nontemporal_store(i32x2{0, 0}, reinterpret_cast<i32x2 *>(pd + 128) + lane);
                __builtin_nontemporal_store((uint16_t)0, reinterpret_cast<uint16_t *>(bd + 128) + lane);
            }
        } else if (c == 0) {
            p3_half<IMG, ROLE, 0, WORDS, STREAM>(L.addr, ga, gb, own4, a.pp, interior, some4, lane, s_hist, s_bkt, bd, pd, wd, a.junk + junk, ablate_flags(a.ablate), pos4, has);
        } else {
            p3_half<IMG, ROLE, 1, WORDS, STREAM>(L.addr, ga, gb, own4, a.pp, interior, some4, lane, s_hist, s_bkt, bd, pd, wd, a.junk + junk, ablate_flags(a.ablate), pos4, has);
        }
    }

    if (more) {
        asm volatile("" : "+v"(own_nxt[0]), "+v"(own_nxt[1]), "+v"(st_halo.v));
        if (STREAM) asm volatile("" : "+v"(pos_nxt[0]), "+v"(pos_nxt[1]));
        p3_unpack_own<C16>(own_nxt[0]), p3_unpack_own<C16>(own_nxt[1]);
        uint32_t nxt_img = IMG ^ 1;
        asm volatile("" : "+s"(nxt_img));
        uint8_t *nxt = lds.cells[0] + nxt_img * kP3ImageBytes;
        uint32_t *nxt_masks = &lds.masks[0][0][0] + nxt_img * (kPredSlots * 16);
        float m = 0.f;
#pragma unroll
        for (int c = 0; c < 2; c++) {
            m = __builtin_fmaxf(m, p3_commit4<CHECK>(raw_own[c], own_nxt[c], nxt + (slot_a + c) * kP3SlotBytes, L.opos[0], L.opos[1]));
            if (ROLE == 1 && lane < 16) nxt_masks[(slot_a + c) * 16 + lane] = st_own_mask[c];
        }
        m = __builtin_fmaxf(m, p3_commit_halo<CHECK>(st_halo, nxt, L.halo_lds));
        if (CHECK) p3_check(m, lane, a.inexact);
    }
    if (tid < kPredSlots) lds.ring[(it + 2) % 3][tid] = slot_pre;
    lds_barrier();
    trace_stamp(a.trace, blockIdx.x, 2 + it, tid);
}

template <int ROLE, bool CHECK, bool WORDS, bool C16 = false, bool STREAM = false>
__device__ __forceinline__ void p3_run(const PredArgs &a, P3Lds &lds, int tid, int lane, int wave, uint32_t &early_poll) {
    uint8_t *s_cells = lds.cells[0];
    int32_t *s_ring = &lds.ring[0][0];
    uint32_t *s_masks = &lds.masks[0][0][0];
    const int pair = wave >> 1;
    const int slot_a = (1 + (pair >> 1)) * kPredSide + 1 + 2 * (pair & 1);
    const int32_t *plane = a.coefs;

    P3Lane L;
    const uint32_t cells_lds = (uint32_t)(uintptr_t)(__attribute__((address_space(3))) uint8_t *)s_cells;
#pragma unroll
    for (int j = 0; j < 4; j++) {
        const u32x4 o = reinterpret_cast<const u32x4 *>(a.pred_off)[p3_node_of<ROLE>(lane, j)];
        const uint32_t rel[3] = {o.x, o.y, o.z};
#pragma unroll
        for (int k = 0; k < 6; k++) {
            const int r = (int)(short)((rel[k >> 1] >> (16 * (k & 1))) & 0xFFFFu);
            L.addr[j][k] = r == 0x7FFF ? cells_lds + kP3ZeroOff : cells_lds + (uint32_t)(slot_a * kP3SlotBytes + r);
        }
    }
    L.opos[0] = 4u * a.pair_pos[ROLE ? 128 + 2 * lane : lane];
    L.opos[1] = 4u * a.pair_pos[ROLE ? 129 + 2 * lane : 64 + lane];
    {
        const uint32_t e = a.halo_list[tid];
        L.halo_ring = 4u * (e & 63u), L.halo_heap = 4u * ((e >> 8) & 511u), L.halo_lds = (e & 63u) * (uint32_t)kP3SlotBytes + (e >> 20);
    }
    float ga[6] = {0.f, 0.f, 0.f, 0.f, 0.f, 0.f}, gb[6] = {0.f, 0.f, 0.f, 0.f, 0.f, 0.f};
    i32x4 own_a[2] = {i32x4{0, 0, 0, 0}, i32x4{0, 0, 0, 0}}, own_b[2] = {i32x4{0, 0, 0, 0}, i32x4{0, 0, 0, 0}};
    u32x4 pos_a[2] = {u32x4{0, 0, 0, 0}, u32x4{0, 0, 0, 0}}, pos_b[2] = {u32x4{0, 0, 0, 0}, u32x4{0, 0, 0, 0}};

    const PredTileWalk walk(a.n_tiles);
    if (walk.first >= walk.end) {
        wait_for_own_memory_ops_then_barrier();
        pred_clear_publish(a, tid);
        return;
    }
    const uint32_t last = walk.first + ((walk.end - 1 - walk.first) / walk.step) * walk.step;
    constexpr uint32_t kLfTilesPerPass = kP3Threads / 2 / 32;
    const uint32_t my_tiles = (walk.end - walk.first + walk.step - 1u) / walk.step;
    const int lf_tid = (wave >> 1) * 64 + lane;
    P3LfItem lf_item;
    if (ROLE == 1) p3_lf_hop_a(a, walk.first + (uint32_t)(lf_tid >> 5) * walk.step, (uint32_t)(lf_tid >> 5) < my_tiles, lf_tid, lf_item);
    if (tid < kPredSlots) {
        s_ring[tid] = a.pred_slots[(size_t)walk.first * kPredSlots + tid];
        s_ring[kPredSlots + tid] = a.pred_slots[(size_t)min(walk.first + walk.step, last) * kPredSlots + tid];
    }
    wait_for_own_memory_ops_then_barrier();
    pred_clear_publish(a, tid);
    {
        uint32_t st_own_mask[2] = {0, 0};
        int raw_own[2];
#pragma unroll
        for (int c = 0; c < 2; c++) {
            raw_own[c] = __builtin_amdgcn_readfirstlane(s_ring[slot_a + c]);
            const int cell = max(pred_slot_cell(raw_own[c]), 0);
            own_a[c] = p3_load_own<ROLE, C16>(plane, (size_t)cell, (uint32_t)lane);
            if (STREAM) pos_a[c] = p3_load_pos<ROLE>(a.stream_pos, (size_t)cell, (uint32_t)lane);
            if (ROLE == 1) st_own_mask[c] = (a.valid_mask + (size_t)cell * 16)[(uint32_t)lane & 15u];
        }
        P3Halo st_halo;
        p3_issue_halo<C16>(plane, s_ring, L.halo_ring, L.halo_heap, st_halo);
        P3LfValues lf_values;
        if (ROLE == 1) p3_lf_hop_b<C16>(a, plane, lf_item, lf_values);
        p3_unpack_own<C16>(own_a[0]), p3_unpack_own<C16>(own_a[1]);
        float m = 0.f;
#pragma unroll
        for (int c = 0; c < 2; c++) {
            m = __builtin_fmaxf(m, p3_commit4<CHECK>(raw_own[c], own_a[c], s_cells + (slot_a + c) * kP3SlotBytes, L.opos[0], L.opos[1]));
            if (ROLE == 1 && lane < 16) s_masks[(slot_a + c) * 16 + lane] = st_own_mask[c];
        }
        m = __builtin_fmaxf(m, p3_commit_halo<CHECK>(st_halo, s_cells, L.halo_lds));
        if (CHECK) p3_check(m, lane, a.inexact);
        if (ROLE == 1 && !(ablate_flags(a.ablate) & 1)) p3_lf_finish<WORDS, STREAM>(a, lds.hist, lf_item, lf_values);
    }
    if (ROLE == 1) {
        for (uint32_t base = kLfTilesPerPass; base < my_tiles; base += kLfTilesPerPass) {
            const uint32_t k = base + (uint32_t)(lf_tid >> 5);
            P3LfItem it;
            P3LfValues x;
            p3_lf_hop_a(a, walk.first + k * walk.step, k < my_tiles, lf_tid, it);
            p3_lf_hop_b<C16>(a, plane, it, x);
            if (!(ablate_flags(a.ablate) & 1)) p3_lf_finish<WORDS, STREAM>(a, lds.hist, it, x);
        }
    }
    lds_barrier();
    trace_stamp(a.trace, blockIdx.x, 1, tid);
    early_poll = pred_clear_poll(a, lane);

    int it = 0;
    for (uint32_t tile = walk.first; tile < walk.end;) {
        p3_tile<0, ROLE, CHECK, WORDS, C16, STREAM>(a, plane, lds, it, tile + walk.step < walk.end, min(tile + 2 * walk.step, last), tid, lane, wave, slot_a, L, ga, gb, own_a, own_b, pos_a, pos_b);
        tile += walk.step, it++;
        if (tile >= walk.end) break;
        p3_tile<1, ROLE, CHECK, WORDS, C16, STREAM>(a, plane, lds, it, tile + walk.step < walk.end, min(tile + 2 * walk.step, last), tid, lane, wave, slot_a, L, ga, gb, own_b, own_a, pos_b, pos_a);
        tile += walk.step, it++;
    }
}

__device__ __forceinline__ PredArgs pred_plane_view(const PredArgs &a0, uint32_t plane) {
    PredArgs a = a0;
    a.coefs += plane * a0.coef_stride;
    if (a.bucket) a.bucket += plane * a0.out_stride;
    if (a.prediction) a.prediction += plane * a0.out_stride;
    if (a.words) a.words += plane * a0.out_stride;
    a.hist += (size_t)plane * kHistBins;
    a.n_oob += plane;
    a.acc += (size_t)plane * kPredAccWords;
    a.inexact = a.acc + kAccInexact;
    if (a0.params)
        a.pp = a0.params[plane];
    else if (plane == 0)
        a.pp = a0.pp3[0];
    else if (plane == 1)
        a.pp = a0.pp3[1];
    else
        a.pp = a0.pp3[2];
    return a;
}

template <bool CHECK, bool WORDS, bool C16 = false, bool STREAM = false>
__global__ void __launch_bounds__(kP3Threads) predict_histogram_kernel3(const PredArgs a0) {
    PredArgs a = pred_plane_view(a0, blockIdx.y);
    if (C16) a.coefs = reinterpret_cast<const int32_t *>(reinterpret_cast<const int16_t *>(a0.coefs) + blockIdx.y * a0.coef_stride);
    __shared__ __attribute__((aligned(16))) P3Lds lds;
    uint32_t *s_hist = lds.hist;
    uint8_t *s_cells = lds.cells[0];
    int32_t *s_ring = &lds.ring[0][0];
    uint16_t *s_bkt = lds.bkt;
    const int tid = threadIdx.x, lane = tid & 63;
    const int wave = __builtin_amdgcn_readfirstlane(tid >> 6);
    trace_stamp(a.trace, blockIdx.x, 0, tid);
    pred_clear_issue(a, tid, kP3Threads);
    for (int i = tid; i < kHistBins + 4; i += kP3Threads) s_hist[i] = 0;
    if (tid < 32) s_bkt[tid] = (uint16_t)(bucket_of((uint32_t)tid) << 12);
    for (int i = tid; i < 2 * (kP3ImageBytes - kP3ZeroOff) / 4; i += kP3Threads)
        reinterpret_cast<uint32_t *>(s_cells + (i / ((kP3ImageBytes - kP3ZeroOff) / 4)) * kP3ImageBytes + kP3ZeroOff)[i % ((kP3ImageBytes - kP3ZeroOff) / 4)] = 0;
    uint32_t early_poll = 0;
    if (wave & 1)
        p3_run<1, CHECK, WORDS, C16, STREAM>(a, lds, tid, lane, wave, early_poll);
    else
        p3_run<0, CHECK, WORDS, C16, STREAM>(a, lds, tid, lane, wave, early_poll);
    lds_barrier();
    trace_stamp(a.trace, blockIdx.x, 13, tid);
    pred_hand_over<CHECK>(a, s_hist, reinterpret_cast<uint32_t *>(s_ring), tid, kP3Threads, early_poll);
    trace_exit(a.trace, blockIdx.x, tid);
}

}


void build_lf_deltas(const uint16_t *nbr_table, int8_t *out ) {
    for (int node = 0; node < 2; node++)
        for (int k = 0; k < 3; k++) {
            const uint32_t e = nbr_table[node * 6 + k];
            const int s7 = (e >> 9) & 7;
            const int da = (int)((0x0F14u >> (2 * s7)) & 3u), db = (int)((0x14F0u >> (2 * s7)) & 3u);
            out[node * 3 + k] = (e & 0x8000u) ? (int8_t)kLfNever : (int8_t)(((da & 1) - (da & 2)) * kPredSide + ((db & 1) - (db & 2)));
        }
    out[6] = out[7] = 0;
}

void build_gather_tables(const uint16_t *nbr_table, uint32_t *gather_off , uint16_t *pair_pos , uint16_t *heap_of_pos ) {
    static const uint16_t kPairPos[256] = {
#include "gather_layout.inc"
    };
    for (int q = 0; q < 256; q++) {
        pair_pos[q] = kPairPos[q];
        heap_of_pos[2 * kPairPos[q]] = (uint16_t)(2 * q);
        heap_of_pos[2 * kPairPos[q] + 1] = (uint16_t)(2 * q + 1);
    }
    for (int p = 0; p < kCell; p++) {
        uint32_t h[6];
        for (int k = 0; k < 6; k++) {
            const uint32_t e = nbr_table[p * 6 + k];
            const int slot = (e >> 9) & 7;
            const int da = (int)((0x0F14u >> (2 * slot)) & 3u), db = (int)((0x14F0u >> (2 * slot)) & 3u);
            const int sa = (da & 1) - (da & 2), sb = (db & 1) - (db & 2);
            const int heap = (int)(e & 511u);
            const int rel = (sa * kPredSide + sb) * 1024 + 2 * (2 * kPairPos[heap >> 1] + (heap & 1));
            h[k] = (e & 0x8000u) ? 0x7FFFu : ((uint32_t)rel & 0xFFFFu);
        }
        gather_off[4 * p] = h[0] | (h[1] << 16), gather_off[4 * p + 1] = h[2] | (h[3] << 16), gather_off[4 * p + 2] = h[4] | (h[5] << 16), gather_off[4 * p + 3] = 0;
    }
}

void build_halo_list(const uint16_t *nbr_table, const uint16_t *pair_pos, uint32_t *out ) {
    std::vector<uint32_t> keys;
    for (int r = 1; r <= kPredBlock; r++)
        for (int c = 1; c <= kPredBlock; c++)
            for (int p = 2; p < kCell; p++)
                for (int k = 0; k < 6; k++) {
                    const uint32_t e = nbr_table[p * 6 + k];
                    const int slot7 = (e >> 9) & 7;
                    if ((e & 0x8000u) || slot7 == 0) continue;
// ... 6 lines not shown
    keys.erase(std::unique(keys.begin(), keys.end()), keys.end());
    out[0] = 0xFFFFFFFFu;
    if (keys.size() > (size_t)kP3Threads) return;
    for (size_t t = keys.size(); t < (size_t)kP3Threads; t++) out[t] = (uint32_t)((t - keys.size()) & 511u) << 8 | (uint32_t)(2 * (t - keys.size())) << 20;
    for (size_t i = 0; i < keys.size(); i++) {
        const uint32_t slot = keys[i] >> 16, heap = keys[i] & 511u;
        const uint32_t pos = 2u * (2u * pair_pos[heap >> 1] + (heap & 1u));
        out[i] = slot | heap << 8 | pos << 20;
    }
}

hipError_t launch_predict_histogram(const DevicePlan &p, uint32_t *acc, uint32_t serial, const PredBatch &b, uint8_t *bucket, int32_t *prediction, uint32_t *hist,
                                    unsigned long long *n_oob, int trust, hipStream_t stream) {
    if (!acc || !serial || !b.n_planes || b.n_planes > 65535u) return hipErrorInvalidValue;
    hipError_t e = hipSuccess;
    PredArgs a{};
    a.acc = acc;
    a.serial = serial;
    for (int k = 0; k < 8; k++) a.lf_delta[k] = p.lf_delta[k];
    if (b.coefs16 && !(b.words && trust == kPredForwardOutput)) return hipErrorInvalidValue;
    a.coefs = b.coefs16 ? reinterpret_cast<const int32_t *>(b.coefs16) : b.coefs;
    a.coef_stride = b.coef_stride;
    a.out_stride = b.out_stride;
    a.params = b.params;
    for (int k = 0; k < 3; k++) a.pp3[k] = b.pp[k];
    a.pred_slots = p.pred_slots;
    a.nbr_table = p.nbr_table;
    a.interior = p.interior;
    a.valid_mask = p.valid_mask;
    a.bucket = bucket;
    a.prediction = prediction;
    a.hist = hist;
    a.n_oob = n_oob;
    a.n_tiles = p.n_pred_tiles;
    a.trusted = trust != kPredAnyInt32 ? 1 : 0;
    a.words = b.words;
    if (b.words && trust != kPredForwardOutput) return hipErrorInvalidValue;
    uint32_t blocks = p.n_pred_tiles < p.pred_blocks ? p.n_pred_tiles : p.pred_blocks;
    if (b.n_planes > 1) {
        const uint32_t share = (p.n_pred_tiles + 7) / 8, eighth = p.pred_blocks / 8 ? p.pred_blocks / 8 : 1;
        blocks = share < eighth ? eighth : share;
        if (blocks > p.pred_blocks) blocks = p.pred_blocks;
        if (blocks > p.n_pred_tiles) blocks = p.n_pred_tiles;
    }
    if (!blocks) blocks = 1;
    a.junk = p.junk;
    a.trace = p.trace;
    a.pred_off = p.gather_off;
    a.pair_pos = p.pair_pos;
    a.heap_of_pos = p.heap_of_pos;
    a.halo_list = p.halo_list;
    a.ablate = p.k2_ablate;
    (void)hipGetLastError();
    a.stream_pos = b.stream_pos;
    if (b.stream_pos && !(b.words && b.coefs16)) return hipErrorInvalidValue;
    if (b.words && b.coefs16 && b.stream_pos)
        hipLaunchKernelGGL((predict_histogram_kernel3<false, true, true, true>), dim3(blocks, b.n_planes), dim3(kP3Threads), 0, stream, a);
    else if (b.words && b.coefs16)
        hipLaunchKernelGGL((predict_histogram_kernel3<false, true, true>), dim3(blocks, b.n_planes), dim3(kP3Threads), 0, stream, a);
    else if (b.words)
        hipLaunchKernelGGL((predict_histogram_kernel3<false, true>), dim3(blocks, b.n_planes), dim3(kP3Threads), 0, stream, a);
    else if (trust == kPredForwardOutput)
        hipLaunchKernelGGL((predict_histogram_kernel3<false, false>), dim3(blocks, b.n_planes), dim3(kP3Threads), 0, stream, a);
    else
        hipLaunchKernelGGL((predict_histogram_kernel3<true, false>), dim3(blocks, b.n_planes), dim3(kP3Threads), 0, stream, a);
    e = hipGetLastError();
    if (e != hipSuccess || trust != kPredAnyInt32) return e;
    ExactArgs x{};
    x.coefs = b.coefs;
    x.coef_stride = b.coef_stride;
    x.out_stride = b.out_stride;
    x.params = b.params;
    for (int k = 0; k < 3; k++) x.pp3[k] = b.pp[k];
    x.nbr_table = p.nbr_table;
    x.nbr_cells = p.nbr_cells;
    x.interior = p.interior;
    x.valid_mask = p.valid_mask;
    x.bucket = bucket;
    x.prediction = prediction;
    x.hist = hist;
    x.n_oob = n_oob;
    x.acc = acc;
    x.F = p.F;
    const uint32_t xb = p.F < blocks ? p.F : blocks;
    (void)hipGetLastError();
    hipLaunchKernelGGL(exact_predict_kernel, dim3(xb ? xb : 1, b.n_planes), dim3(kCell), 0, stream, x);
    return hipGetLastError();
}

}
```

### frave_amd/csrc/kernels.hpp

```cpp
#pragma once
#include <hip/hip_runtime_api.h>

#include <cstddef>
#include <cstdint>

#include "geometry.hpp"

namespace fri {

struct DevicePlan {
    const Tile *tiles = nullptr;
    const int32_t *tile_cells = nullptr;
    const TileCell *tile_meta = nullptr;
    const int32_t *wg_tiles = nullptr;
    const int32_t *wg_tiles_batch = nullptr;
    uint32_t n_wg_batch = 0;
    uint32_t n_wg = 0;
    int32_t max_tile_cells = 0;
    bool covers_image = false;
    int32_t max_wg_tiles = 0;
    int32_t max_wg_cells = 0;
    int32_t inv_group = 1;
    int32_t inv_max_wg_tiles = 0, inv_max_wg_cells = 0;
    const Int2 *centers = nullptr;
    const uint8_t *interior = nullptr;
    const uint32_t *valid_mask = nullptr;
    const int32_t *nbr_cells = nullptr;
    const uint16_t *nbr_table = nullptr;
    const uint32_t *gather_off = nullptr;
    const uint16_t *pair_pos = nullptr;
    const uint16_t *heap_of_pos = nullptr;
    const uint32_t *halo_list = nullptr;
    int8_t lf_delta[8] = {0, 0, 0, 0, 0, 0, 0, 0};
    const int32_t *pred_slots = nullptr;
    uint32_t n_pred_tiles = 0;
    uint32_t *hist_partial = nullptr;
    unsigned long long *oob_partial = nullptr;
    uint32_t hist_blocks = 0;
    uint8_t *junk = nullptr;
    uint32_t pred_blocks = 0;
    uint32_t n_tiles = 0;
    uint32_t F = 0;
    int32_t width = 0, height = 0, channels = 0;
    int32_t lds_pitch = 0, lds_rows = 0, cells_per_tile = 0;
    bool k1_batch_shares = true;
    int k1_cached_stores = -1;
    int32_t k1_ablate = 0;
    int32_t k2_ablate = 0;
    bool rct = false;
    bool ycc = false;
    bool k3_multiply = false;
    bool k3_midpoint = false;
    unsigned long long *trace = nullptr;
    bool k1_measuring = false;
    unsigned long long *k1_xcd_stat = nullptr;
    const InvTileLists *inv_lists = nullptr;
    const uint16_t *inv_quads = nullptr, *inv_dwords = nullptr;
    const uint32_t *inv_parts = nullptr;
    int32_t inv_rect_bytes = 0;
    bool k3_scan = false;
    int32_t k3_ablate = 0;
    int32_t k4_ablate = 0;
    int32_t k4_older_eighths = 5;
};

constexpr uint32_t kPredJunkWaves = 16, kPredJunkBytes = 2560;
constexpr uint32_t kFitAccWords = 3 * 28 + 18 + 2;
constexpr uint32_t kFitShards = 16;
constexpr uint32_t kPredAccRing = 8, kPredAccWords = 16;

struct QMatrix {
    int32_t q[32];
};

struct PredictParams {
    float value[3][6];
    float width[3][6];
};

hipError_t launch_fwd_transform_quant(const DevicePlan &p, uint32_t n_images, const uint8_t *pixels, size_t pixel_stride, int32_t *coefs,
                                      size_t coef_stride, const QMatrix &q, hipStream_t stream, bool cached_stores = false,
                                      int16_t *coefs16 = nullptr );
struct PredBatch {
    uint32_t n_planes = 1;
    const int32_t *coefs = nullptr;
    const int16_t *coefs16 = nullptr;
    size_t coef_stride = 0, out_stride = 0;
    const PredictParams *params = nullptr;
    PredictParams pp[3] = {};
    const uint32_t *stream_pos = nullptr;
    uint16_t *words = nullptr;
};
constexpr int kPredAnyInt32 = 0, kPredPromised = 1, kPredForwardOutput = 2;
hipError_t launch_predict_histogram(const DevicePlan &p, uint32_t *acc, uint32_t serial, const PredBatch &b, uint8_t *bucket, int32_t *prediction, uint32_t *hist,
                                    unsigned long long *n_oob, int trust, hipStream_t stream);
struct FitSolve {
    float *params = nullptr;
    float *host_params = nullptr;
    unsigned long long *host_range = nullptr;
    unsigned long long rows[3] = {0, 0, 0};
};
hipError_t launch_fit_accumulate(const DevicePlan &p, unsigned long long *acc, int mode, const PredBatch &b, unsigned long long *sums_int, double *sums_dbl,
                                 unsigned long long *out_of_range, hipStream_t stream, const FitSolve *solve = nullptr, int trust = 0 );
hipError_t launch_fit_solve(int mode, uint32_t n_planes, const unsigned long long *sums_int, const double *sums_dbl, const unsigned long long rows[3], float *params,
                            hipStream_t stream, float *host_params = nullptr, const unsigned long long *range = nullptr, unsigned long long *host_range = nullptr);
hipError_t launch_inverse_transform(const DevicePlan &p, uint32_t n_images, const int32_t *coefs, size_t coef_stride, const QMatrix &q, uint8_t *pixels, size_t pixel_stride,
                                    hipStream_t stream, unsigned long long *measure = nullptr);

hipError_t launch_symbol_gather(const uint32_t *order, uint64_t n_symbols, uint32_t n_planes, const uint16_t *words, size_t word_stride, uint16_t *out, size_t stream_stride,
                                hipStream_t stream);
hipError_t launch_symbol_stream(const uint32_t *order, uint64_t n_symbols, uint32_t n_planes, const int32_t *coefs, size_t coef_stride, const uint8_t *bucket,
                                const int32_t *prediction, size_t out_stride, uint16_t *out, size_t stream_stride, hipStream_t stream);

struct RateLayout {
    uint32_t header_bytes, channel_bytes, context_bytes;
};
hipError_t launch_rate_estimate(uint32_t n_images, uint32_t channels, const uint32_t *hist, const unsigned long long *oob, const float *laplace,
                                unsigned long long *bytes, uint32_t *models, const RateLayout &layout, hipStream_t stream);
hipError_t launch_rate_estimate_tiled(uint32_t n_tiles, uint32_t channels, const uint32_t *hist, const unsigned long long *oob, const float *laplace,
                                      unsigned long long *tile_bytes, unsigned long long *file_bytes, uint32_t *models, const RateLayout &layout, hipStream_t stream);

hipError_t launch_rate_estimate_tiled420(uint32_t n_tiles, const uint32_t *hist, const unsigned long long *oob, const float *laplace, unsigned long long *tile_bytes,
                                         unsigned long long *file_bytes, uint32_t *models, const RateLayout &layout, hipStream_t stream);

hipError_t launch_ssim(uint32_t n_images, const uint8_t *a, const uint8_t *b, size_t pixel_stride, uint32_t width, uint32_t height, uint32_t channels,
                       unsigned long long *out, hipStream_t stream);

hipError_t launch_clear_sums(unsigned long long *sums, uint32_t n, hipStream_t stream);
hipError_t launch_split420(const uint8_t *rgb, uint32_t width, uint32_t height, uint8_t *y, uint8_t *cbcr, hipStream_t stream);
hipError_t launch_merge420(const uint8_t *y, const uint8_t *cbcr, uint32_t width, uint32_t height, uint8_t *rgb, hipStream_t stream, unsigned long long *measure = nullptr);

hipError_t launch_split_rgba(const uint8_t *rgba, uint32_t width, uint32_t height, bool clean, uint8_t *rgb, uint8_t *a, hipStream_t stream);
hipError_t launch_merge_rgba(const uint8_t *rgb, const uint8_t *a, uint32_t width, uint32_t height, uint8_t *rgba, hipStream_t stream);

hipError_t launch_split_tiles(const uint8_t *image, uint32_t width, uint32_t height, uint32_t channels, uint32_t tile_w, uint32_t tile_h, uint8_t *tiles, hipStream_t stream);
hipError_t launch_merge_tiles(const uint8_t *tiles, uint32_t width, uint32_t height, uint32_t channels, uint32_t tile_w, uint32_t tile_h, uint8_t *image, hipStream_t stream);
hipError_t launch_merge_tiles_region(const uint8_t *tiles, uint32_t width, uint32_t height, uint32_t channels, uint32_t tile_w, uint32_t tile_h, uint32_t x, uint32_t y, uint32_t w,
                                     uint32_t h, uint8_t *region, hipStream_t stream);
hipError_t launch_merge_tiles_regions(const uint8_t *tiles, uint32_t channels, uint32_t tile_w, uint32_t tile_h, uint32_t nx, uint32_t n_regions, uint32_t n_groups,
                                      const uint32_t *table, uint8_t *out, hipStream_t stream);
hipError_t launch_split_tiles_region(const uint8_t *src, size_t src_pitch, uint32_t src_x, uint32_t src_y, uint32_t src_w, uint32_t src_h, uint32_t width, uint32_t height,
                                     uint32_t channels, uint32_t tile_w, uint32_t tile_h, uint32_t x, uint32_t y, uint32_t w, uint32_t h, uint8_t *tiles, hipStream_t stream);
hipError_t launch_measure_tiles(const uint8_t *tiles, uint32_t width, uint32_t height, uint32_t channels, uint32_t tile_w, uint32_t tile_h, const uint8_t *reference,
// ... 46 lines not shown
```

### include/fri_hip.h

```cpp
#ifndef FRI_HIP_H
#define FRI_HIP_H

#include <stddef.h>
#include <stdint.h>

#ifdef __cplusplus
extern "C" {
#endif
#if defined(__GNUC__)
#pragma GCC visibility push(default)
#endif

#define FRI_HIP_NONE INT32_MIN
#define FRI_HIP_CELL_SIZE 512
#define FRI_HIP_CONTEXT_AMOUNT 10
#define FRI_HIP_ALPHABET_SIZE 1024

#define FRI_HIP_OK 0
#define FRI_HIP_ERR_INVALID_ARGUMENT (-1)
#define FRI_HIP_ERR_HIP (-2)
#define FRI_HIP_ERR_NO_DEVICE (-3)
#define FRI_HIP_ERR_OUT_OF_MEMORY (-4)
#define FRI_HIP_ERR_DIVIDE_BY_ZERO (-5)
#define FRI_HIP_ERR_EMPTY_LATTICE (-6)
// ... 49 lines not shown
                                  int32_t *const *coefs);

int fri_hip_predict_histogram(fri_hip_plan *plan, const int32_t *coefs, uint32_t channel, const float value_params[3][6],
                              const float width_params[3][6], uint8_t *bucket, int32_t *prediction, uint32_t *hist,
                              uint64_t *n_out_of_alphabet);
int fri_hip_plan_assume_forward_coefficients(fri_hip_plan *plan, int on);
int fri_hip_predict_histogram_dev(fri_hip_plan *plan, const int32_t *d_coefs, uint32_t channel, const float value_params[3][6],
                                  const float width_params[3][6], uint8_t *d_bucket, int32_t *d_prediction, uint32_t *d_hist,
                                  uint64_t *d_n_out_of_alphabet, void *stream);

int fri_hip_predict_histogram_batch_dev(fri_hip_plan *plan, uint32_t n_planes, const int32_t *d_coefs, size_t coef_stride, const float *d_params, uint8_t *d_bucket,
                                        int32_t *d_prediction, size_t out_stride, uint32_t *d_hist, uint64_t *d_n_out_of_alphabet, void *stream);

int fri_hip_fit_value_sums(fri_hip_plan *plan, const int32_t *coefs, uint32_t channel, int64_t gram[3][28]);
int fri_hip_fit_value_sums_dev(fri_hip_plan *plan, const int32_t *d_coefs, uint32_t channel, int64_t *d_gram, void *stream);
int fri_hip_fit_width_sums(fri_hip_plan *plan, const int32_t *coefs, uint32_t channel, const float value_params[3][6], int64_t wtw[3][21],
                           double wtr[3][6], uint64_t rows[3]);
int fri_hip_fit_width_sums_dev(fri_hip_plan *plan, const int32_t *d_coefs, uint32_t channel, const float value_params[3][6], int64_t *d_wtw,
                               double *d_wtr, void *stream);

int fri_hip_fit_value_sums_batch_dev(fri_hip_plan *plan, uint32_t n_planes, const int32_t *d_coefs, size_t coef_stride, int64_t *d_gram, void *stream);
int fri_hip_fit_width_sums_batch_dev(fri_hip_plan *plan, uint32_t n_planes, const int32_t *d_coefs, size_t coef_stride, const float *d_params, int64_t *d_wtw, double *d_wtr,
                                     void *stream);
void fri_hip_solve6(const double m[6][6], const double y[6], double x[6]);
void fri_hip_fit_value_params(const int64_t gram[3][28], float value_params[3][6]);
void fri_hip_fit_width_params(const int64_t wtw[3][21], const double wtr[3][6], const uint64_t rows[3], float width_params[3][6]);

int fri_hip_fit_value_params_batch_dev(fri_hip_plan *plan, uint32_t n_planes, const int64_t *d_gram, float *d_params, void *stream);
int fri_hip_fit_width_params_batch_dev(fri_hip_plan *plan, uint32_t n_planes, const int64_t *d_wtw, const double *d_wtr, float *d_params, void *stream);

int fri_hip_fit_params_batch_dev(fri_hip_plan *plan, uint32_t n_planes, const int32_t *d_coefs, size_t coef_stride, float *d_params, uint64_t *d_fit_out_of_range,
                                 void *stream);

int fri_hip_encode_image(fri_hip_plan *plan, const uint8_t *pixels, const int32_t qmatrix[32], int fit, float *value_params, float *width_params, int32_t *coefs,
                         uint8_t *bucket, int32_t *prediction, uint32_t *hist, uint64_t *n_out_of_alphabet);
int fri_hip_encode_image_dev(fri_hip_plan *plan, const uint8_t *d_pixels, const int32_t qmatrix[32], int fit, float *value_params, float *width_params, int32_t *d_coefs,
                             uint8_t *d_bucket, int32_t *d_prediction, uint32_t *d_hist, uint64_t *d_n_out_of_alphabet, void *stream);

int fri_hip_encode_image_batch_dev(fri_hip_plan *plan, uint32_t n_images, const uint8_t *d_pixels, size_t pixel_stride, const int32_t qmatrix[32], int fit, float *d_params,
                                   int32_t *d_coefs, size_t coef_stride, uint8_t *d_bucket, int32_t *d_prediction, size_t out_stride, uint32_t *d_hist,
                                   uint64_t *d_n_out_of_alphabet, uint64_t *d_fit_out_of_range, void *stream);

int fri_hip_encode_image_batch(fri_hip_plan *plan, uint32_t n_images, const uint8_t *const *pixels, const int32_t qmatrix[32], int fit, float *const *params,
                               int32_t *const *coefs, uint8_t *const *bucket, int32_t *const *prediction, uint32_t *const *hist, uint64_t *const *n_out_of_alphabet);
int fri_hip_multi_encode_image(fri_hip_multi *m, uint32_t n_images, const uint8_t *const *pixels, const int32_t qmatrix[32], int fit, float *const *params,
                               int32_t *const *coefs, uint8_t *const *bucket, int32_t *const *prediction, uint32_t *const *hist, uint64_t *const *n_out_of_alphabet);

int fri_hip_predict_image(fri_hip_plan *plan, const int32_t *coefs, int fit, float *value_params, float *width_params, uint8_t *bucket, int32_t *prediction,
                          uint32_t *hist, uint64_t *n_out_of_alphabet);
int fri_hip_predict_image_dev(fri_hip_plan *plan, const int32_t *d_coefs, int fit, float *value_params, float *width_params, uint8_t *d_bucket, int32_t *d_prediction,
                              uint32_t *d_hist, uint64_t *d_n_out_of_alphabet, void *stream);

int fri_hip_plan_set_stream_order(fri_hip_plan *plan, const uint32_t *order, uint64_t n);
int fri_hip_symbol_stream_batch_dev(fri_hip_plan *plan, uint32_t n_planes, const int32_t *d_coefs, size_t coef_stride, const uint8_t *d_bucket, const int32_t *d_prediction,
                                    size_t out_stride, uint16_t *d_symbols, size_t symbol_stride, void *stream);

int fri_hip_encode_symbols_batch_dev(fri_hip_plan *plan, uint32_t n_images, const uint8_t *d_pixels, size_t pixel_stride, const int32_t qmatrix[32], int fit, float *d_params,
                                     int32_t *d_coefs, size_t coef_stride, uint16_t *d_node_words, size_t word_stride, uint16_t *d_symbols, size_t symbol_stride,
                                     uint32_t *d_hist, uint64_t *d_n_out_of_alphabet, uint64_t *d_fit_out_of_range, void *stream);

int fri_hip_encode_image_symbols(fri_hip_plan *plan, const uint8_t *pixels, const int32_t qmatrix[32], int fit, float *value_params, float *width_params, uint16_t *symbols,
                                 uint32_t *hist, uint64_t *n_out_of_alphabet);

int fri_hip_inverse_transform(fri_hip_plan *plan, const int32_t *coefs, const int32_t qmatrix[32], uint8_t *pixels);
#define FRI_HIP_DEQUANT_REFERENCE 0
#define FRI_HIP_DEQUANT_MULTIPLY 1
#define FRI_HIP_DEQUANT_MIDPOINT 2
int fri_hip_plan_set_dequantiser(fri_hip_plan *plan, int mode);

int fri_hip_quality_matrix(int quality, int32_t qmatrix[32]);
int fri_hip_measure_distortion_dev(fri_hip_plan *plan, const int32_t *d_coefs, const int32_t qmatrix[32], const uint8_t *d_reference_pixels, uint64_t *d_out,
                                   void *stream);
int fri_hip_search_quality(fri_hip_plan *plan, const uint8_t *pixels, double target_db, int32_t *quality, double *psnr_db);
int fri_hip_search_quality_dev(fri_hip_plan *plan, const uint8_t *d_pixels, double target_db, int32_t *quality, double *psnr_db, void *stream);
int fri_hip_estimate_size_dev(fri_hip_plan *plan, uint32_t n_images, const uint32_t *d_hist, const uint64_t *d_n_out_of_alphabet, uint64_t *d_bytes, uint32_t *d_models,
                              void *stream);
int fri_hip_estimate_size(fri_hip_plan *plan, const uint32_t *hist, const uint64_t *n_out_of_alphabet, uint64_t *bytes);
int fri_hip_search_quality_for_size(fri_hip_plan *plan, const uint8_t *pixels, uint64_t max_bytes, int32_t *quality, uint64_t *est_bytes);
int fri_hip_search_quality_for_size_dev(fri_hip_plan *plan, const uint8_t *d_pixels, uint64_t max_bytes, int32_t *quality, uint64_t *est_bytes, void *stream);
int fri_hip_measure_ssim_dev(fri_hip_plan *plan, uint32_t n_images, const uint8_t *d_a, const uint8_t *d_b, size_t pixel_stride, int64_t *d_out, void *stream);
int fri_hip_measure_ssim(fri_hip_plan *plan, const uint8_t *a, const uint8_t *b, int64_t *out);
int fri_hip_search_quality_ssim(fri_hip_plan *plan, const uint8_t *pixels, double target, int32_t *quality, double *ssim);
int fri_hip_search_quality_ssim_dev(fri_hip_plan *plan, const uint8_t *d_pixels, double target, int32_t *quality, double *ssim, void *stream);
#define FRI_HIP_COLOUR_NONE 0
#define FRI_HIP_COLOUR_RCT 1
#define FRI_HIP_COLOUR_YCBCR 3
int fri_hip_plan_set_colour_transform(fri_hip_plan *plan, int mode);
int fri_hip_inverse_transform_dev(fri_hip_plan *plan, const int32_t *d_coefs, const int32_t qmatrix[32], uint8_t *d_pixels,
                                  void *stream);
int fri_hip_inverse_transform_batch_dev(fri_hip_plan *plan, uint32_t n_images, const int32_t *d_coefs, size_t coef_stride, const int32_t qmatrix[32], uint8_t *d_pixels,
                                        size_t pixel_stride, void *stream);

typedef struct fri_hip_plan420 fri_hip_plan420;
int fri_hip_plan420_create(fri_hip_ctx *ctx, uint32_t width, uint32_t height, fri_hip_plan420 **out);
int fri_hip_plan420_destroy(fri_hip_plan420 *p);
fri_hip_plan *fri_hip_plan420_luma(fri_hip_plan420 *p);
fri_hip_plan *fri_hip_plan420_chroma(fri_hip_plan420 *p);
int fri_hip_split420_dev(fri_hip_plan420 *p, const uint8_t *d_rgb, uint8_t *d_y, uint8_t *d_cbcr, void *stream);
int fri_hip_merge420_dev(fri_hip_plan420 *p, const uint8_t *d_y, const uint8_t *d_cbcr, uint8_t *d_rgb, void *stream);
int fri_hip_measure_distortion420_dev(fri_hip_plan420 *p, const uint8_t *d_y, const uint8_t *d_cbcr, const uint8_t *d_reference_rgb, uint64_t *d_out, void *stream);
int fri_hip_encode_image420_symbols(fri_hip_plan420 *p, const uint8_t *pixels, int quality, float *value_params, float *width_params, uint16_t *symbols, uint32_t *hist,
                                    uint64_t *n_out_of_alphabet);
int fri_hip_decode_image420(fri_hip_plan420 *p, const int32_t *coefs, int quality, uint8_t *pixels);
int fri_hip_search_quality420(fri_hip_plan420 *p, const uint8_t *pixels, double target_db, int32_t *quality, double *psnr_db);
int fri_hip_search_quality420_dev(fri_hip_plan420 *p, const uint8_t *d_pixels, double target_db, int32_t *quality, double *psnr_db, void *stream);
int fri_hip_search_quality_for_size420(fri_hip_plan420 *p, const uint8_t *pixels, uint64_t max_bytes, int32_t *quality, uint64_t *est_bytes);
// ... 189 lines not shown
```

### integration/hip_sys.rs

```rust
#![allow(non_camel_case_types, dead_code)]
use std::os::raw::{c_char, c_int, c_void};

#[repr(C)] pub struct fri_hip_ctx { _private: [u8; 0] }
#[repr(C)] pub struct fri_hip_plan { _private: [u8; 0] }
#[repr(C)] pub struct fri_hip_multi { _private: [u8; 0] }
#[repr(C)] pub struct fri_hip_plan420 { _private: [u8; 0] }
#[repr(C)] pub struct fri_hip_plan_rgba { _private: [u8; 0] }
#[repr(C)] pub struct fri_hip_plan_tiled { _private: [u8; 0] }
#[repr(C)] pub struct fri_hip_plan_tiled420 { _private: [u8; 0] }
#[repr(C)] pub struct fri_hip_plan_tiled_rgba { _private: [u8; 0] }

pub const FRI_HIP_NONE: i32 = i32::MIN;
pub const FRI_HIP_OK: c_int = 0;
pub const FRI_HIP_ERR_INVALID_ARGUMENT: c_int = -1;
pub const FRI_HIP_ERR_HIP: c_int = -2;
pub const FRI_HIP_ERR_NO_DEVICE: c_int = -3;
pub const FRI_HIP_ERR_OUT_OF_MEMORY: c_int = -4;
pub const FRI_HIP_ERR_DIVIDE_BY_ZERO: c_int = -5;
pub const FRI_HIP_ERR_EMPTY_LATTICE: c_int = -6;
pub const FRI_HIP_ERR_OUT_OF_RANGE: c_int = -7;

#[link(name = "fri_hip")]
extern "C" {
    pub fn fri_hip_strerror(code: c_int) -> *const c_char;
// ... 4 lines not shown
    pub fn fri_hip_last_hip_error(ctx: *const fri_hip_ctx) -> *const c_char;
    pub fn fri_hip_plan_create(ctx: *mut fri_hip_ctx, width: u32, height: u32, channels: u32, out: *mut *mut fri_hip_plan) -> c_int;
    pub fn fri_hip_plan_destroy(plan: *mut fri_hip_plan) -> c_int;
    pub fn fri_hip_plan_num_cells(plan: *const fri_hip_plan) -> u32;
    pub fn fri_hip_plan_num_bfs_cells(plan: *const fri_hip_plan) -> u32;
    pub fn fri_hip_plan_num_interior_cells(plan: *const fri_hip_plan) -> u32;
    pub fn fri_hip_plan_coef_count(plan: *const fri_hip_plan) -> usize;
    pub fn fri_hip_plan_pixel_bytes(plan: *const fri_hip_plan) -> usize;
    pub fn fri_hip_plan_centers(plan: *const fri_hip_plan, centers: *mut i32) -> c_int;
    pub fn fri_hip_plan_valid_mask(plan: *const fri_hip_plan, mask: *mut u32) -> c_int;
    pub fn fri_hip_plan_num_some(plan: *const fri_hip_plan) -> u64;
    pub fn fri_hip_plan_num_some_levels(plan: *const fri_hip_plan, levels: u32, out: *mut u64) -> c_int;
    pub fn fri_hip_plan_neighbour_cells(plan: *const fri_hip_plan, ids: *mut i32) -> c_int;
    pub fn fri_hip_plan_neighbour_table(plan: *const fri_hip_plan, table: *mut u16) -> c_int;
    pub fn fri_hip_plan_tiling(plan: *const fri_hip_plan, out: *mut i32) -> c_int;
    pub fn fri_hip_plan_predict_grid(plan: *const fri_hip_plan, out: *mut u32) -> c_int;
    pub fn fri_hip_plan_pred_slots(plan: *const fri_hip_plan, out: *mut i32) -> c_int;
    pub fn fri_hip_plan_tile_table(plan: *const fri_hip_plan, tiles: *mut i32, tile_cells: *mut i32, wg_tiles: *mut i32) -> c_int;
    pub fn fri_hip_transform_quant(plan: *mut fri_hip_plan, pixels: *const u8, qmatrix: *const i32, coefs: *mut i32) -> c_int;
    pub fn fri_hip_transform_quant_dev(plan: *mut fri_hip_plan, d_pixels: *const u8, qmatrix: *const i32, d_coefs: *mut i32, stream: *mut c_void) -> c_int;
    pub fn fri_hip_transform_quant_batch_dev(plan: *mut fri_hip_plan, n_images: u32, d_pixels: *const u8, pixel_stride: usize, qmatrix: *const i32, d_coefs: *mut i32, coef_stride: usize, stream: *mut c_void) -> c_int;
    pub fn fri_hip_transform_quant_batch(plan: *mut fri_hip_plan, n_images: u32, pixels: *const *const u8, qmatrix: *const i32, coefs: *const *mut i32) -> c_int;
    pub fn fri_hip_shard_size(n_images: u32, shard: u32, n_shards: u32) -> u32;
    pub fn fri_hip_shard_image(k: u32, shard: u32, n_shards: u32) -> u32;
    pub fn fri_hip_multi_create(devices: *const c_int, n_devices: u32, width: u32, height: u32, channels: u32, out: *mut *mut fri_hip_multi) -> c_int;
    pub fn fri_hip_multi_destroy(m: *mut fri_hip_multi) -> c_int;
    pub fn fri_hip_multi_num_devices(m: *const fri_hip_multi) -> u32;
    pub fn fri_hip_multi_plan(m: *mut fri_hip_multi, d: u32) -> *mut fri_hip_plan;
    pub fn fri_hip_multi_transform_quant(m: *mut fri_hip_multi, n_images: u32, pixels: *const *const u8, qmatrix: *const i32, coefs: *const *mut i32) -> c_int;
    pub fn fri_hip_predict_histogram(plan: *mut fri_hip_plan, coefs: *const i32, channel: u32, value_params: *const [f32; 6], width_params: *const [f32; 6], bucket: *mut u8, prediction: *mut i32, hist: *mut u32, n_out_of_alphabet: *mut u64) -> c_int;
    pub fn fri_hip_plan_assume_forward_coefficients(plan: *mut fri_hip_plan, on: c_int) -> c_int;
    pub fn fri_hip_predict_histogram_dev(plan: *mut fri_hip_plan, d_coefs: *const i32, channel: u32, value_params: *const [f32; 6], width_params: *const [f32; 6], d_bucket: *mut u8, d_prediction: *mut i32, d_hist: *mut u32, d_n_out_of_alphabet: *mut u64, stream: *mut c_void) -> c_int;
    pub fn fri_hip_predict_histogram_batch_dev(plan: *mut fri_hip_plan, n_planes: u32, d_coefs: *const i32, coef_stride: usize, d_params: *const f32, d_bucket: *mut u8, d_prediction: *mut i32, out_stride: usize, d_hist: *mut u32, d_n_out_of_alphabet: *mut u64, stream: *mut c_void) -> c_int;
    pub fn fri_hip_fit_value_sums(plan: *mut fri_hip_plan, coefs: *const i32, channel: u32, gram: *mut [i64; 28]) -> c_int;
    pub fn fri_hip_fit_value_sums_dev(plan: *mut fri_hip_plan, d_coefs: *const i32, channel: u32, d_gram: *mut i64, stream: *mut c_void) -> c_int;
    pub fn fri_hip_fit_width_sums(plan: *mut fri_hip_plan, coefs: *const i32, channel: u32, value_params: *const [f32; 6], wtw: *mut [i64; 21], wtr: *mut [f64; 6], rows: *mut u64) -> c_int;
    pub fn fri_hip_fit_width_sums_dev(plan: *mut fri_hip_plan, d_coefs: *const i32, channel: u32, value_params: *const [f32; 6], d_wtw: *mut i64, d_wtr: *mut f64, stream: *mut c_void) -> c_int;
    pub fn fri_hip_fit_value_sums_batch_dev(plan: *mut fri_hip_plan, n_planes: u32, d_coefs: *const i32, coef_stride: usize, d_gram: *mut i64, stream: *mut c_void) -> c_int;
    pub fn fri_hip_fit_width_sums_batch_dev(plan: *mut fri_hip_plan, n_planes: u32, d_coefs: *const i32, coef_stride: usize, d_params: *const f32, d_wtw: *mut i64, d_wtr: *mut f64, stream: *mut c_void) -> c_int;
    pub fn fri_hip_solve6(m: *const [f64; 6], y: *const f64, x: *mut f64);
    pub fn fri_hip_fit_value_params(gram: *const [i64; 28], value_params: *mut [f32; 6]);
    pub fn fri_hip_fit_width_params(wtw: *const [i64; 21], wtr: *const [f64; 6], rows: *const u64, width_params: *mut [f32; 6]);
    pub fn fri_hip_fit_value_params_batch_dev(plan: *mut fri_hip_plan, n_planes: u32, d_gram: *const i64, d_params: *mut f32, stream: *mut c_void) -> c_int;
    pub fn fri_hip_fit_width_params_batch_dev(plan: *mut fri_hip_plan, n_planes: u32, d_wtw: *const i64, d_wtr: *const f64, d_params: *mut f32, stream: *mut c_void) -> c_int;
    pub fn fri_hip_fit_params_batch_dev(plan: *mut fri_hip_plan, n_planes: u32, d_coefs: *const i32, coef_stride: usize, d_params: *mut f32, d_fit_out_of_range: *mut u64, stream: *mut c_void) -> c_int;
    pub fn fri_hip_encode_image(plan: *mut fri_hip_plan, pixels: *const u8, qmatrix: *const i32, fit: c_int, value_params: *mut f32, width_params: *mut f32, coefs: *mut i32, bucket: *mut u8, prediction: *mut i32, hist: *mut u32, n_out_of_alphabet: *mut u64) -> c_int;
    pub fn fri_hip_encode_image_dev(plan: *mut fri_hip_plan, d_pixels: *const u8, qmatrix: *const i32, fit: c_int, value_params: *mut f32, width_params: *mut f32, d_coefs: *mut i32, d_bucket: *mut u8, d_prediction: *mut i32, d_hist: *mut u32, d_n_out_of_alphabet: *mut u64, stream: *mut c_void) -> c_int;
    pub fn fri_hip_encode_image_batch_dev(plan: *mut fri_hip_plan, n_images: u32, d_pixels: *const u8, pixel_stride: usize, qmatrix: *const i32, fit: c_int, d_params: *mut f32, d_coefs: *mut i32, coef_stride: usize, d_bucket: *mut u8, d_prediction: *mut i32, out_stride: usize, d_hist: *mut u32, d_n_out_of_alphabet: *mut u64, d_fit_out_of_range: *mut u64, stream: *mut c_void) -> c_int;
    pub fn fri_hip_encode_image_batch(plan: *mut fri_hip_plan, n_images: u32, pixels: *const *const u8, qmatrix: *const i32, fit: c_int, params: *const *mut f32, coefs: *const *mut i32, bucket: *const *mut u8, prediction: *const *mut i32, hist: *const *mut u32, n_out_of_alphabet: *const *mut u64) -> c_int;
    pub fn fri_hip_multi_encode_image(m: *mut fri_hip_multi, n_images: u32, pixels: *const *const u8, qmatrix: *const i32, fit: c_int, params: *const *mut f32, coefs: *const *mut i32, bucket: *const *mut u8, prediction: *const *mut i32, hist: *const *mut u32, n_out_of_alphabet: *const *mut u64) -> c_int;
    pub fn fri_hip_predict_image(plan: *mut fri_hip_plan, coefs: *const i32, fit: c_int, value_params: *mut f32, width_params: *mut f32, bucket: *mut u8, prediction: *mut i32, hist: *mut u32, n_out_of_alphabet: *mut u64) -> c_int;
    pub fn fri_hip_predict_image_dev(plan: *mut fri_hip_plan, d_coefs: *const i32, fit: c_int, value_params: *mut f32, width_params: *mut f32, d_bucket: *mut u8, d_prediction: *mut i32, d_hist: *mut u32, d_n_out_of_alphabet: *mut u64, stream: *mut c_void) -> c_int;
    pub fn fri_hip_plan_set_stream_order(plan: *mut fri_hip_plan, order: *const u32, n: u64) -> c_int;
    pub fn fri_hip_symbol_stream_batch_dev(plan: *mut fri_hip_plan, n_planes: u32, d_coefs: *const i32, coef_stride: usize, d_bucket: *const u8, d_prediction: *const i32, out_stride: usize, d_symbols: *mut u16, symbol_stride: usize, stream: *mut c_void) -> c_int;
    pub fn fri_hip_encode_symbols_batch_dev(plan: *mut fri_hip_plan, n_images: u32, d_pixels: *const u8, pixel_stride: usize, qmatrix: *const i32, fit: c_int, d_params: *mut f32, d_coefs: *mut i32, coef_stride: usize, d_node_words: *mut u16, word_stride: usize, d_symbols: *mut u16, symbol_stride: usize, d_hist: *mut u32, d_n_out_of_alphabet: *mut u64, d_fit_out_of_range: *mut u64, stream: *mut c_void) -> c_int;
    pub fn fri_hip_encode_image_symbols(plan: *mut fri_hip_plan, pixels: *const u8, qmatrix: *const i32, fit: c_int, value_params: *mut f32, width_params: *mut f32, symbols: *mut u16, hist: *mut u32, n_out_of_alphabet: *mut u64) -> c_int;
    pub fn fri_hip_inverse_transform(plan: *mut fri_hip_plan, coefs: *const i32, qmatrix: *const i32, pixels: *mut u8) -> c_int;
    pub fn fri_hip_plan_set_dequantiser(plan: *mut fri_hip_plan, mode: c_int) -> c_int;
    pub fn fri_hip_quality_matrix(quality: c_int, qmatrix: *mut i32) -> c_int;
    pub fn fri_hip_measure_distortion_dev(plan: *mut fri_hip_plan, d_coefs: *const i32, qmatrix: *const i32, d_reference_pixels: *const u8, d_out: *mut u64, stream: *mut c_void) -> c_int;
    pub fn fri_hip_search_quality(plan: *mut fri_hip_plan, pixels: *const u8, target_db: f64, quality: *mut i32, psnr_db: *mut f64) -> c_int;
    pub fn fri_hip_search_quality_dev(plan: *mut fri_hip_plan, d_pixels: *const u8, target_db: f64, quality: *mut i32, psnr_db: *mut f64, stream: *mut c_void) -> c_int;
    pub fn fri_hip_estimate_size_dev(plan: *mut fri_hip_plan, n_images: u32, d_hist: *const u32, d_n_out_of_alphabet: *const u64, d_bytes: *mut u64, d_models: *mut u32, stream: *mut c_void) -> c_int;
    pub fn fri_hip_estimate_size(plan: *mut fri_hip_plan, hist: *const u32, n_out_of_alphabet: *const u64, bytes: *mut u64) -> c_int;
    pub fn fri_hip_search_quality_for_size(plan: *mut fri_hip_plan, pixels: *const u8, max_bytes: u64, quality: *mut i32, est_bytes: *mut u64) -> c_int;
    pub fn fri_hip_search_quality_for_size_dev(plan: *mut fri_hip_plan, d_pixels: *const u8, max_bytes: u64, quality: *mut i32, est_bytes: *mut u64, stream: *mut c_void) -> c_int;
    pub fn fri_hip_measure_ssim_dev(plan: *mut fri_hip_plan, n_images: u32, d_a: *const u8, d_b: *const u8, pixel_stride: usize, d_out: *mut i64, stream: *mut c_void) -> c_int;
    pub fn fri_hip_measure_ssim(plan: *mut fri_hip_plan, a: *const u8, b: *const u8, out: *mut i64) -> c_int;
    pub fn fri_hip_search_quality_ssim(plan: *mut fri_hip_plan, pixels: *const u8, target: f64, quality: *mut i32, ssim: *mut f64) -> c_int;
    pub fn fri_hip_search_quality_ssim_dev(plan: *mut fri_hip_plan, d_pixels: *const u8, target: f64, quality: *mut i32, ssim: *mut f64, stream: *mut c_void) -> c_int;
    pub fn fri_hip_plan_set_colour_transform(plan: *mut fri_hip_plan, mode: c_int) -> c_int;
    pub fn fri_hip_inverse_transform_dev(plan: *mut fri_hip_plan, d_coefs: *const i32, qmatrix: *const i32, d_pixels: *mut u8, stream: *mut c_void) -> c_int;
    pub fn fri_hip_inverse_transform_batch_dev(plan: *mut fri_hip_plan, n_images: u32, d_coefs: *const i32, coef_stride: usize, qmatrix: *const i32, d_pixels: *mut u8, pixel_stride: usize, stream: *mut c_void) -> c_int;
    pub fn fri_hip_plan420_create(ctx: *mut fri_hip_ctx, width: u32, height: u32, out: *mut *mut fri_hip_plan420) -> c_int;
    pub fn fri_hip_plan420_destroy(p: *mut fri_hip_plan420) -> c_int;
    pub fn fri_hip_plan420_luma(p: *mut fri_hip_plan420) -> *mut fri_hip_plan;
    pub fn fri_hip_plan420_chroma(p: *mut fri_hip_plan420) -> *mut fri_hip_plan;
    pub fn fri_hip_split420_dev(p: *mut fri_hip_plan420, d_rgb: *const u8, d_y: *mut u8, d_cbcr: *mut u8, stream: *mut c_void) -> c_int;
    pub fn fri_hip_merge420_dev(p: *mut fri_hip_plan420, d_y: *const u8, d_cbcr: *const u8, d_rgb: *mut u8, stream: *mut c_void) -> c_int;
    pub fn fri_hip_measure_distortion420_dev(p: *mut fri_hip_plan420, d_y: *const u8, d_cbcr: *const u8, d_reference_rgb: *const u8, d_out: *mut u64, stream: *mut c_void) -> c_int;
    pub fn fri_hip_encode_image420_symbols(p: *mut fri_hip_plan420, pixels: *const u8, quality: c_int, value_params: *mut f32, width_params: *mut f32, symbols: *mut u16, hist: *mut u32, n_out_of_alphabet: *mut u64) -> c_int;
    pub fn fri_hip_decode_image420(p: *mut fri_hip_plan420, coefs: *const i32, quality: c_int, pixels: *mut u8) -> c_int;
    pub fn fri_hip_search_quality420(p: *mut fri_hip_plan420, pixels: *const u8, target_db: f64, quality: *mut i32, psnr_db: *mut f64) -> c_int;
    pub fn fri_hip_search_quality420_dev(p: *mut fri_hip_plan420, d_pixels: *const u8, target_db: f64, quality: *mut i32, psnr_db: *mut f64, stream: *mut c_void) -> c_int;
    pub fn fri_hip_search_quality_for_size420(p: *mut fri_hip_plan420, pixels: *const u8, max_bytes: u64, quality: *mut i32, est_bytes: *mut u64) -> c_int;
    pub fn fri_hip_search_quality_for_size420_dev(p: *mut fri_hip_plan420, d_pixels: *const u8, max_bytes: u64, quality: *mut i32, est_bytes: *mut u64, stream: *mut c_void) -> c_int;
    pub fn fri_hip_search_quality_ssim420(p: *mut fri_hip_plan420, pixels: *const u8, target: f64, quality: *mut i32, ssim: *mut f64) -> c_int;
    pub fn fri_hip_search_quality_ssim420_dev(p: *mut fri_hip_plan420, d_pixels: *const u8, target: f64, quality: *mut i32, ssim: *mut f64, stream: *mut c_void) -> c_int;
    pub fn fri_hip_plan_rgba_create(ctx: *mut fri_hip_ctx, width: u32, height: u32, out: *mut *mut fri_hip_plan_rgba) -> c_int;
    pub fn fri_hip_plan_rgba_destroy(p: *mut fri_hip_plan_rgba) -> c_int;
    pub fn fri_hip_plan_rgba_colour(p: *mut fri_hip_plan_rgba) -> *mut fri_hip_plan;
    pub fn fri_hip_plan_rgba_alpha(p: *mut fri_hip_plan_rgba) -> *mut fri_hip_plan;
    pub fn fri_hip_split_rgba_dev(p: *mut fri_hip_plan_rgba, d_rgba: *const u8, clean: c_int, d_rgb: *mut u8, d_a: *mut u8, stream: *mut c_void) -> c_int;
    pub fn fri_hip_merge_rgba_dev(p: *mut fri_hip_plan_rgba, d_rgb: *const u8, d_a: *const u8, d_rgba: *mut u8, stream: *mut c_void) -> c_int;
    pub fn fri_hip_encode_symbols_rgba_dev(p: *mut fri_hip_plan_rgba, d_rgba: *const u8, clean: c_int, qmatrix: *const i32, fit: c_int, d_params: *mut f32, d_symbols: *mut u16, d_hist: *mut u32, d_n_out_of_alphabet: *mut u64, d_fit_out_of_range: *mut u64, stream: *mut c_void) -> c_int;
    pub fn fri_hip_encode_image_rgba_symbols(p: *mut fri_hip_plan_rgba, pixels: *const u8, clean: c_int, qmatrix: *const i32, value_params: *mut f32, width_params: *mut f32, symbols: *mut u16, hist: *mut u32, n_out_of_alphabet: *mut u64) -> c_int;
    pub fn fri_hip_decode_image_rgba(p: *mut fri_hip_plan_rgba, coefs: *const i32, qmatrix: *const i32, pixels: *mut u8) -> c_int;
    pub fn fri_hip_plan_owned_pixels(plan: *const fri_hip_plan) -> u64;
    pub fn fri_hip_tile_shape(width: u32, height: u32, target: u32, tile_w: *mut u32, tile_h: *mut u32) -> c_int;
    pub fn fri_hip_plan_tiled_create(ctx: *mut fri_hip_ctx, width: u32, height: u32, channels: u32, tile_w: u32, tile_h: u32, flags: u32, out: *mut *mut fri_hip_plan_tiled) -> c_int;
    pub fn fri_hip_plan_tiled_destroy(p: *mut fri_hip_plan_tiled) -> c_int;
    pub fn fri_hip_plan_tiled_tile(p: *mut fri_hip_plan_tiled) -> *mut fri_hip_plan;
    pub fn fri_hip_plan_tiled_grid(p: *const fri_hip_plan_tiled, out: *mut u32) -> c_int;
    pub fn fri_hip_split_tiles_dev(p: *mut fri_hip_plan_tiled, d_raster: *const u8, d_tiles: *mut u8, stream: *mut c_void) -> c_int;
    pub fn fri_hip_merge_tiles_dev(p: *mut fri_hip_plan_tiled, d_tiles: *const u8, d_raster: *mut u8, stream: *mut c_void) -> c_int;
    pub fn fri_hip_encode_symbols_tiled_dev(p: *mut fri_hip_plan_tiled, d_raster: *const u8, qmatrix: *const i32, fit: c_int, d_params: *mut f32, d_symbols: *mut u16, d_hist: *mut u32, d_n_out_of_alphabet: *mut u64, d_fit_out_of_range: *mut u64, stream: *mut c_void) -> c_int;
// ... 86 lines not shown
```

Before: 910,700.

## Compact stream position table to 16-bit offsets plus per-group bases

Replaces the 32-bit per-node stream position table used by the predict kernel's direct symbol-stream output with per-cell group bases and 16-bit offsets, selected when every offset fits in 16 bits. This halves the bytes of position data the predict kernel loads per cell, at the cost of an extra base lookup and add. It also adds an API to query the format and compute the compact tables, plus an env switch to force the 32-bit path. The measured transform+quant encode path likely does not use stream positions, so it is probably unaffected.

Result: slower. 900,800 (-1.1%).

```diff
diff --git a/frave_amd/api.py b/frave_amd/api.py
--- a/frave_amd/api.py
+++ b/frave_amd/api.py
@@ -24,7 +24,7 @@
     "fri_hip_encode_image_dev", "fri_hip_inverse_transform_batch_dev", "fri_hip_predict_image", "fri_hip_predict_image_dev",
     "fri_hip_fit_params_batch_dev", "fri_hip_encode_image_batch_dev", "fri_hip_fit_value_params_batch_dev", "fri_hip_fit_width_params_batch_dev",
     "fri_hip_plan_assume_forward_coefficients", "fri_hip_encode_image_batch", "fri_hip_multi_encode_image",
-    "fri_hip_plan_set_stream_order", "fri_hip_symbol_stream_batch_dev", "fri_hip_encode_image_symbols", "fri_hip_encode_symbols_batch_dev",
+    "fri_hip_plan_set_stream_order", "fri_hip_plan_stream_position_format", "fri_hip_plan_compact_stream_positions", "fri_hip_symbol_stream_batch_dev", "fri_hip_encode_image_symbols", "fri_hip_encode_symbols_batch_dev",
     "fri_hip_plan_set_dequantiser", "fri_hip_plan_tune_forward", "fri_hip_time_transform_quant_streams_dev",
     "fri_hip_plan_set_colour_transform", "fri_hip_quality_matrix", "fri_hip_measure_distortion_dev", "fri_hip_search_quality",
     "fri_hip_search_quality_dev", "fri_hip_estimate_size_dev", "fri_hip_estimate_size", "fri_hip_search_quality_for_size",
@@ -190,6 +190,8 @@
     L.fri_hip_search_quality_ssim.argtypes = [vp, vp, C.c_double, vp, vp]
     L.fri_hip_search_quality_ssim_dev.argtypes = [vp, vp, C.c_double, vp, vp, vp]
     L.fri_hip_plan_set_stream_order.argtypes = [vp, vp, C.c_uint64]
+    L.fri_hip_plan_stream_position_format.argtypes = [vp]
+    L.fri_hip_plan_compact_stream_positions.argtypes = [vp, vp, C.c_uint64, vp, vp, vp, vp]
     L.fri_hip_symbol_stream_batch_dev.argtypes = [vp, u32, vp, sz, vp, vp, sz, vp, sz, vp]
     L.fri_hip_encode_image_symbols.argtypes = [vp, vp, vp, i32, vp, vp, vp, vp, vp]
     L.fri_hip_encode_symbols_batch_dev.argtypes = [vp, u32, vp, sz, vp, i32, vp, vp, sz, vp, sz, vp, sz, vp, vp, vp, vp]
@@ -614,6 +616,18 @@
         _check(load_library().fri_hip_plan_set_stream_order(self._h, _p(order), order.size), "fri_hip_plan_set_stream_order", self.ctx)
         return order
 
+    def stream_position_format(self):
+        return int(load_library().fri_hip_plan_stream_position_format(self._h))
+
+    def compact_stream_positions(self, order):
+        order = np.ascontiguousarray(order, np.uint32)
+        base = np.empty((self.num_cells, 24), np.uint32)
+        off = np.empty((self.num_cells, 512), np.uint16)
+        largest, fmt = C.c_uint32(0), C.c_int(0)
+        _check(load_library().fri_hip_plan_compact_stream_positions(self._h, _p(order), order.size, _p(base), _p(off), C.byref(largest), C.byref(fmt)),
+               "fri_hip_plan_compact_stream_positions", self.ctx)
+        return base, off, int(largest.value), int(fmt.value)
+
     def symbol_stream_batch_dev(self, n_planes, d_coefs, coef_stride, d_bucket, d_prediction, out_stride, d_symbols, symbol_stride, stream=0):
         _check(load_library().fri_hip_symbol_stream_batch_dev(self._h, n_planes, d_coefs, coef_stride, d_bucket, d_prediction, out_stride, d_symbols, symbol_stride, stream),
                "fri_hip_symbol_stream_batch_dev", self.ctx)
diff --git a/frave_amd/csrc/fri_hip.cpp b/frave_amd/csrc/fri_hip.cpp
--- a/frave_amd/csrc/fri_hip.cpp
+++ b/frave_amd/csrc/fri_hip.cpp
@@ -58,6 +58,7 @@
     int inv_band_rows = 0;
     int pred_blocks = 0, hist_blocks = 0, trace = 0, k3_scan = 0;
     int k1_ablate = 0, k2_ablate = 0, k3_ablate = 0, k4_ablate = 0;
+    int stream_pos32 = 0;
     std::optional<int> k1_cached_stores, k1_batch_shares, k4_older_eighths;
 };
 
@@ -84,6 +85,7 @@
     k.inv_shared = opt(env("FRI_HIP_INV_SHARED")), k.inv_strided_shares = opt(env("FRI_HIP_INV_STRIDED_SHARES")), k.inv_band_rows = num(env("FRI_HIP_INV_BAND_ROWS"));
     k.pred_blocks = num(env("FRI_HIP_PRED_BLOCKS")), k.hist_blocks = num(env("FRI_HIP_HIST_BLOCKS")), k.trace = num(env("FRI_HIP_TRACE")), k.k3_scan = num(env("FRI_HIP_K3_SCAN"));
     k.k1_ablate = num(env("FRI_HIP_K1_ABLATE")), k.k2_ablate = num(env("FRI_HIP_K2_ABLATE")), k.k3_ablate = num(env("FRI_HIP_K3_ABLATE")), k.k4_ablate = num(env("FRI_HIP_K4_ABLATE"));
+    k.stream_pos32 = num(env("FRI_HIP_STREAM_POS32"));
     k.k1_cached_stores = opt(env("FRI_HIP_K1_CACHED_STORES")), k.k1_batch_shares = opt(env("FRI_HIP_K1_BATCH_SHARES")), k.k4_older_eighths = opt(env("FRI_HIP_K4_OLDER_EIGHTHS"));
     return k;
 }
@@ -607,6 +609,7 @@
     if (k.k1_cached_stores) d.k1_cached_stores = *k.k1_cached_stores > 0 ? 1 : 0;
     if (k.k1_batch_shares) d.k1_batch_shares = *k.k1_batch_shares != 0;
     d.k2_ablate = k.k2_ablate;
+    p->stream_pos32 = k.stream_pos32 > 0;
     d.k3_ablate = k.k3_ablate;
     d.k3_scan = k.k3_scan > 0;
     d.k4_ablate = k.k4_ablate;
@@ -1092,6 +1095,9 @@
     return fit_launch(p, 1, b, (int64_t *)k.sums_int.get(), k.sums_dbl, nullptr, s, &solve, trust);
 }
 
+static void set_stream_positions(PredBatch &b, const fri_hip_plan *p) {
+    b.stream_pos = p->d_stream_pos, b.stream_off = p->d_stream_off, b.stream_base = p->d_stream_base, b.stream_len = (uint32_t)p->geo.n_some;
+}
 static int predict_image_dev(fri_hip_plan *p, const int32_t *d_coefs, int fit, float *value_params, float *width_params, uint8_t *d_bucket, int32_t *d_prediction,
                              uint32_t *d_hist, uint64_t *d_oob, int trust, hipStream_t s, uint16_t *d_words = nullptr, const int16_t *d_coefs16 = nullptr,
                              uint16_t *d_streams = nullptr) {
@@ -1105,7 +1111,7 @@
     b.coef_stride = plane;
     b.out_stride = plane;
     b.words = d_words;
-    if (d_streams) b.words = d_streams, b.out_stride = p->geo.n_some, b.stream_pos = p->d_stream_pos;
+    if (d_streams) b.words = d_streams, b.out_stride = p->geo.n_some, set_stream_positions(b, p);
     if (!fit) {
         for (uint32_t ch = 0; ch < C; ch++) {
             std::memcpy(b.pp[ch].value, value_params + ch * 18, sizeof(b.pp[ch].value));
@@ -1211,7 +1217,7 @@
     b.out_stride = C > 1 ? plane : word_stride;
     b.params = reinterpret_cast<const PredictParams *>(d_params);
     b.words = d_node_words;
-    if (direct) b.words = d_symbols, b.out_stride = C > 1 ? n : symbol_stride, b.stream_pos = p->d_stream_pos;
+    if (direct) b.words = d_symbols, b.out_stride = C > 1 ? n : symbol_stride, set_stream_positions(b, p);
     if (fit)
         if (int rc = fit_chain(p, b, (unsigned long long *)d_fit_out_of_range, s, nullptr, nullptr, kPredForwardOutput)) return rc;
     if (int rc = predict_launch(p, b, nullptr, nullptr, d_hist, d_n_out_of_alphabet, kPredForwardOutput, s)) return rc;
@@ -1373,26 +1379,79 @@
     });
 }
 
-int fri_hip_plan_set_stream_order(fri_hip_plan *p, const uint32_t *order, uint64_t n) {
-    if (int rc = need_device(p)) return rc;
-    if (!order || n != p->geo.n_some) return FRI_HIP_ERR_INVALID_ARGUMENT;
+namespace {
+bool is_stream_order(const fri_hip_plan *p, const uint32_t *order, uint64_t n) {
+    if (!order || n != p->geo.n_some) return false;
     const size_t F = p->geo.centers.size();
     std::vector<uint8_t> seen(F * kCell, 0);
     for (uint64_t i = 0; i < n; i++) {
         const uint32_t e = order[i], cell = e >> 9, heap = e & 511u;
-        if (cell >= F || !((p->geo.valid_mask[(size_t)cell * 16 + (heap >> 5)] >> (heap & 31)) & 1u) || seen[e]) return FRI_HIP_ERR_INVALID_ARGUMENT;
+        if (cell >= F || !((p->geo.valid_mask[(size_t)cell * 16 + (heap >> 5)] >> (heap & 31)) & 1u) || seen[e]) return false;
         seen[e] = 1;
     }
+    return true;
+}
+uint32_t compact_stream_positions(const uint32_t *order, uint64_t n, size_t F, uint32_t *base , uint16_t *off ) {
+    std::fill(base, base + F * kPosGroups, 0xFFFFFFFFu);
+    for (uint64_t i = 0; i < n; i++) {
+        uint32_t &b = base[(size_t)(order[i] >> 9) * kPosGroups + pos_group(order[i] & 511u)];
+        b = std::min(b, (uint32_t)i);
+    }
+    std::fill(off, off + F * kCell, (uint16_t)0);
+    uint32_t largest = 0;
+    for (uint64_t i = 0; i < n; i++) {
+        const uint32_t d = (uint32_t)i - base[(size_t)(order[i] >> 9) * kPosGroups + pos_group(order[i] & 511u)];
+        off[order[i]] = (uint16_t)d;
+        largest = std::max(largest, d);
+    }
+    for (size_t k = 0; k < F * kPosGroups; k++)
+        if (base[k] == 0xFFFFFFFFu) base[k] = 0;
+    return largest;
+}
+
+int stream_position_format(uint32_t largest, bool force32) { return largest <= 0xFFFFu && !force32 ? 16 : 32; }
+}
+
+int fri_hip_plan_compact_stream_positions(const fri_hip_plan *p, const uint32_t *order, uint64_t n, uint32_t *base, uint16_t *offset, uint32_t *largest_offset, int *format) {
+    if (!p || !base || !offset || !largest_offset || !format || !is_stream_order(p, order, n)) return FRI_HIP_ERR_INVALID_ARGUMENT;
+    *largest_offset = compact_stream_positions(order, n, p->geo.centers.size(), base, offset);
+    *format = stream_position_format(*largest_offset, p->stream_pos32);
+    return FRI_HIP_OK;
+}
+
+int fri_hip_plan_stream_position_format(const fri_hip_plan *p) {
+    if (!p || !p->d_stream_order) return 0;
+    return p->d_stream_off ? 16 : 32;
+}
+
+int fri_hip_plan_set_stream_order(fri_hip_plan *p, const uint32_t *order, uint64_t n) {
+    if (int rc = need_device(p)) return rc;
+    if (!is_stream_order(p, order, n)) return FRI_HIP_ERR_INVALID_ARGUMENT;
+    const size_t F = p->geo.centers.size();
     fri_hip_ctx *c = p->ctx;
     HIP_TRY(c, hipSetDevice(c->device));
-    std::vector<uint32_t> pos(F * kCell, 0xFFFFFFFFu);
-    for (uint64_t i = 0; i < n; i++) pos[order[i]] = (uint32_t)i;
-    DevMem<uint32_t> d_order, d_pos;
+    std::vector<uint32_t> base(F * kPosGroups), pos;
+    std::vector<uint16_t> off(F * kCell);
+    const bool compact = stream_position_format(compact_stream_positions(order, n, F, base.data(), off.data()), p->stream_pos32) == 16;
+    if (!compact) {
+        std::vector<uint32_t>().swap(base), std::vector<uint16_t>().swap(off);
+        pos.assign(F * kCell, 0xFFFFFFFFu);
+        for (uint64_t i = 0; i < n; i++) pos[order[i]] = (uint32_t)i;
+    }
+    DevMem<uint32_t> d_order, d_pos, d_base;
+    DevMem<uint16_t> d_off;
     HIP_TRY(c, hipMalloc((void **)d_order.put(), (n ? n : 1) * sizeof(uint32_t)));
     HIP_TRY(c, hipMemcpy(d_order, order, n * sizeof(uint32_t), hipMemcpyHostToDevice));
-    HIP_TRY(c, hipMalloc((void **)d_pos.put(), pos.size() * sizeof(uint32_t)));
-    HIP_TRY(c, hipMemcpy(d_pos, pos.data(), pos.size() * sizeof(uint32_t), hipMemcpyHostToDevice));
-    p->d_stream_order = std::move(d_order), p->d_stream_pos = std::move(d_pos);
+    if (compact) {
+        HIP_TRY(c, hipMalloc((void **)d_base.put(), base.size() * sizeof(uint32_t)));
+        HIP_TRY(c, hipMemcpy(d_base, base.data(), base.size() * sizeof(uint32_t), hipMemcpyHostToDevice));
+        HIP_TRY(c, hipMalloc((void **)d_off.put(), off.size() * sizeof(uint16_t)));
+        HIP_TRY(c, hipMemcpy(d_off, off.data(), off.size() * sizeof(uint16_t), hipMemcpyHostToDevice));
+    } else {
+        HIP_TRY(c, hipMalloc((void **)d_pos.put(), pos.size() * sizeof(uint32_t)));
+        HIP_TRY(c, hipMemcpy(d_pos, pos.data(), pos.size() * sizeof(uint32_t), hipMemcpyHostToDevice));
+    }
+    p->d_stream_order = std::move(d_order), p->d_stream_pos = std::move(d_pos), p->d_stream_base = std::move(d_base), p->d_stream_off = std::move(d_off);
     return FRI_HIP_OK;
 }
 
diff --git a/frave_amd/csrc/fri_hip_internal.hpp b/frave_amd/csrc/fri_hip_internal.hpp
--- a/frave_amd/csrc/fri_hip_internal.hpp
+++ b/frave_amd/csrc/fri_hip_internal.hpp
@@ -134,7 +134,9 @@
     const float *laplace = nullptr;
     bool assume_forward = false;
     DevMem<uint32_t> d_stream_order;
-    DevMem<uint32_t> d_stream_pos;
+    DevMem<uint32_t> d_stream_pos, d_stream_base;
+    DevMem<uint16_t> d_stream_off;
+    bool stream_pos32 = false;
     Grown<int16_t> coefs16;
     Event ev_coefs16;
     hipStream_t coefs16_stream = nullptr;
diff --git a/frave_amd/csrc/k2_predict.hip b/frave_amd/csrc/k2_predict.hip
--- a/frave_amd/csrc/k2_predict.hip
+++ b/frave_amd/csrc/k2_predict.hip
@@ -63,6 +63,9 @@
     int32_t trusted;
     PredictParams pp;
     PredictParams pp3[3];
+    const uint16_t *stream_off;
+    const uint32_t *stream_base;
+    uint32_t stream_len;
 };
 
 constexpr int kAccZeroFlag = 0, kAccTicket = 12, kAccInexact = 14;
@@ -336,7 +339,7 @@
     x.value = at(cell);
     x.mask0 = a.valid_mask[(size_t)cell * 16];
 }
-template <bool WORDS, bool STREAM = false>
+template <bool WORDS, bool STREAM = false, bool P16 = false>
 __device__ __forceinline__ void p3_lf_finish(const PredArgs &a, uint32_t *s_hist, const P3LfItem &it, const P3LfValues &x) {
     const int cell = pred_slot_cell(it.raw);
     if (cell < 0) return;
@@ -351,7 +354,8 @@
     const uint32_t counter = sym < 1024u ? (b12 >> 2) + sym : (uint32_t)kHistBins;
     if (some) atomicAdd(&s_hist[counter], 1u);
     if (WORDS && STREAM) {
-        if (some) a.words[a.stream_pos[(size_t)cell * kCell + it.node]] = (uint16_t)counter;
+        if (some && P16) a.words[a.stream_base[(size_t)cell * kPosGroups + it.node] + a.stream_off[(size_t)cell * kCell + it.node]] = (uint16_t)counter;
+        if (some && !P16) a.words[a.stream_pos[(size_t)cell * kCell + it.node]] = (uint16_t)counter;
         return;
     }
     if (WORDS) {
@@ -515,6 +519,7 @@
     uint32_t halo_ring;
     uint32_t halo_heap;
     uint32_t halo_lds;
+    uint32_t pgrp[2];
 };
 
 template <int ROLE, bool C16 = false>
@@ -544,10 +549,64 @@
     return u32x4{(uint32_t)a.x, (uint32_t)a.y, (uint32_t)b.x, (uint32_t)b.y};
 }
 
-template <int IMG, int ROLE, bool CHECK, bool WORDS, bool C16 = false, bool STREAM = false>
+struct P3Pos16 {
+    uint32_t off01, off23;
+    uint32_t base01, base23;
+};
+template <int ROLE>
+__device__ __forceinline__ P3Pos16 p3_load_pos16(const uint16_t *stream_off, const uint32_t *stream_base, size_t cell, uint32_t lane, const uint32_t (&pgrp)[2]) {
+    const uint16_t *off = stream_off + cell * kCell;
+    const uint32_t *base = stream_base + cell * kPosGroups;
+    P3Pos16 r;
+    if (ROLE) {
+        const i32x2 d = reinterpret_cast<const i32x2 *>(off + 256)[lane];
+        r.off01 = (uint32_t)d.x, r.off23 = (uint32_t)d.y, r.base01 = base[pgrp[0]], r.base23 = 0;
+    } else {
+        r.off01 = reinterpret_cast<const uint32_t *>(off)[lane], r.off23 = reinterpret_cast<const uint32_t *>(off + 128)[lane];
+        r.base01 = base[pgrp[0]], r.base23 = base[pgrp[1]];
+    }
+    return r;
+}
+template <int ROLE>
+__device__ __forceinline__ void p3_pos4(const u32x4 &p, uint32_t (&out)[4]) {
+    out[0] = p.x, out[1] = p.y, out[2] = p.z, out[3] = p.w;
+}
+template <int ROLE>
+__device__ __forceinline__ void p3_pos4(const P3Pos16 &p, uint32_t (&out)[4]) {
+    const uint32_t b23 = ROLE ? p.base01 : p.base23;
+    out[0] = p.base01 + (p.off01 & 0xFFFFu), out[1] = p.base01 + (p.off01 >> 16), out[2] = b23 + (p.off23 & 0xFFFFu), out[3] = b23 + (p.off23 >> 16);
+}
+template <int ROLE>
+__device__ __forceinline__ void p3_pin_pos(u32x4 (&p)[2]) {
+    asm volatile("" : "+v"(p[0]), "+v"(p[1]));
+}
+template <int ROLE>
+__device__ __forceinline__ void p3_pin_pos(P3Pos16 (&p)[2]) {
+    asm volatile("" : "+v"(p[0].off01), "+v"(p[0].off23), "+v"(p[0].base01), "+v"(p[1].off01), "+v"(p[1].off23), "+v"(p[1].base01));
+    if (ROLE == 0) asm volatile("" : "+v"(p[0].base23), "+v"(p[1].base23));
+}
+template <bool P16>
+struct P3PosOf {
+    typedef u32x4 type;
+};
+template <>
+struct P3PosOf<true> {
+    typedef P3Pos16 type;
+};
+template <int ROLE>
+__device__ __forceinline__ void p3_ablate_pos(uint32_t cell, int lane, uint32_t stream_len, uint32_t (&out)[4]) {
+#pragma unroll
+    for (int j = 0; j < 4; j++) {
+        const uint32_t at = cell * (uint32_t)kCell + (uint32_t)p3_node_of<ROLE>(lane, j);
+        const uint32_t folded = at - stream_len;
+        out[j] = at < stream_len ? at : folded < stream_len ? folded : 0u;
+    }
+}
+
+template <int IMG, int ROLE, bool CHECK, bool WORDS, bool C16 = false, bool STREAM = false, bool P16 = false>
 __device__ __forceinline__ void p3_tile(const PredArgs &a, const int32_t *plane, P3Lds &lds, int it, bool more, uint32_t next2_tile, int tid, int lane, int wave, int slot_a,
-                                        const P3Lane &L, float (&ga)[6], float (&gb)[6], const i32x4 (&own_cur)[2], i32x4 (&own_nxt)[2], const u32x4 (&pos_cur)[2],
-                                        u32x4 (&pos_nxt)[2]) {
+                                        const P3Lane &L, float (&ga)[6], float (&gb)[6], const i32x4 (&own_cur)[2], i32x4 (&own_nxt)[2],
+                                        const typename P3PosOf<P16>::type (&pos_cur)[2], typename P3PosOf<P16>::type (&pos_nxt)[2]) {
     uint32_t *s_hist = lds.hist;
     const uint16_t *s_bkt = lds.bkt;
     const int32_t *cur_slots = lds.ring[it % 3], *nxt_slots = lds.ring[(it + 1) % 3];
@@ -562,7 +621,12 @@
             raw_own[c] = __builtin_amdgcn_readfirstlane(nxt_slots[slot_a + c]);
             const int cell = max(pred_slot_cell(raw_own[c]), 0);
             own_nxt[c] = p3_load_own<ROLE, C16>(plane, (size_t)cell, (uint32_t)lane);
-            if (STREAM) pos_nxt[c] = p3_load_pos<ROLE>(a.stream_pos, (size_t)cell, (uint32_t)lane);
+            if (STREAM && !(ablate_flags(a.ablate) & 64)) {
+                if constexpr (P16)
+                    pos_nxt[c] = p3_load_pos16<ROLE>(a.stream_off, a.stream_base, (size_t)cell, (uint32_t)lane, L.pgrp);
+                else
+                    pos_nxt[c] = p3_load_pos<ROLE>(a.stream_pos, (size_t)cell, (uint32_t)lane);
+            }
             if (ROLE == 1) st_own_mask[c] = (a.valid_mask + (size_t)cell * 16)[(uint32_t)lane & 15u];
         }
         p3_issue_halo<C16>(plane, nxt_slots, L.halo_ring, L.halo_heap, st_halo);
@@ -577,7 +641,17 @@
         uint8_t *bd = has && a.bucket ? a.bucket + (size_t)cell * kCell : a.junk + junk;
         int32_t *pd = has && a.prediction ? a.prediction + (size_t)cell * kCell : reinterpret_cast<int32_t *>(a.junk + junk + 512);
         uint16_t *wd = WORDS && STREAM ? a.words : WORDS && has ? a.words + (size_t)cell * kCell : reinterpret_cast<uint16_t *>(a.junk + junk + 512);
-        const uint32_t pos4[4] = {pos_cur[c].x, pos_cur[c].y, pos_cur[c].z, pos_cur[c].w};
+        uint32_t pos4[4];
+        p3_pos4<ROLE>(pos_cur[c], pos4);
+        if (STREAM && (ablate_flags(a.ablate) & (64 | 128))) {
+            uint32_t side[4];
+            p3_ablate_pos<ROLE>((uint32_t)max(cell, 0), lane, a.stream_len, side);
+#pragma unroll
+            for (int j = 0; j < 4; j++) {
+                if (ablate_flags(a.ablate) & 128) asm volatile("" ::"v"(pos4[j]));
+                pos4[j] = side[j];
+            }
+        }
         uint32_t some4 = 0;
         if (!interior && has) {
             const uint32_t *m = lds.masks[IMG][slot_a + c];
@@ -615,7 +689,7 @@
 
     if (more) {
         asm volatile("" : "+v"(own_nxt[0]), "+v"(own_nxt[1]), "+v"(st_halo.v));
-        if (STREAM) asm volatile("" : "+v"(pos_nxt[0]), "+v"(pos_nxt[1]));
+        if (STREAM) p3_pin_pos<ROLE>(pos_nxt);
         p3_unpack_own<C16>(own_nxt[0]), p3_unpack_own<C16>(own_nxt[1]);
         uint32_t nxt_img = IMG ^ 1;
         asm volatile("" : "+s"(nxt_img));
@@ -635,7 +709,7 @@
     trace_stamp(a.trace, blockIdx.x, 2 + it, tid);
 }
 
-template <int ROLE, bool CHECK, bool WORDS, bool C16 = false, bool STREAM = false>
+template <int ROLE, bool CHECK, bool WORDS, bool C16 = false, bool STREAM = false, bool P16 = false>
 __device__ __forceinline__ void p3_run(const PredArgs &a, P3Lds &lds, int tid, int lane, int wave, uint32_t &early_poll) {
     uint8_t *s_cells = lds.cells[0];
     int32_t *s_ring = &lds.ring[0][0];
@@ -664,7 +738,12 @@
     }
     float ga[6] = {0.f, 0.f, 0.f, 0.f, 0.f, 0.f}, gb[6] = {0.f, 0.f, 0.f, 0.f, 0.f, 0.f};
     i32x4 own_a[2] = {i32x4{0, 0, 0, 0}, i32x4{0, 0, 0, 0}}, own_b[2] = {i32x4{0, 0, 0, 0}, i32x4{0, 0, 0, 0}};
-    u32x4 pos_a[2] = {u32x4{0, 0, 0, 0}, u32x4{0, 0, 0, 0}}, pos_b[2] = {u32x4{0, 0, 0, 0}, u32x4{0, 0, 0, 0}};
+    typename P3PosOf<P16>::type pos_a[2] = {}, pos_b[2] = {};
+    L.pgrp[0] = L.pgrp[1] = 0;
+    if constexpr (P16) {
+        L.pgrp[0] = ROLE ? 13u + ((uint32_t)lane >> 3) : lane < 32 ? 33u - (uint32_t)__builtin_clz((uint32_t)lane | 1u) : 5u + ((uint32_t)lane >> 4);
+        L.pgrp[1] = ROLE ? L.pgrp[0] : 9u + ((uint32_t)lane >> 4);
+    }
 
     const PredTileWalk walk(a.n_tiles);
     if (walk.first >= walk.end) {
@@ -692,7 +771,12 @@
             raw_own[c] = __builtin_amdgcn_readfirstlane(s_ring[slot_a + c]);
             const int cell = max(pred_slot_cell(raw_own[c]), 0);
             own_a[c] = p3_load_own<ROLE, C16>(plane, (size_t)cell, (uint32_t)lane);
-            if (STREAM) pos_a[c] = p3_load_pos<ROLE>(a.stream_pos, (size_t)cell, (uint32_t)lane);
+            if (STREAM && !(ablate_flags(a.ablate) & 64)) {
+                if constexpr (P16)
+                    pos_a[c] = p3_load_pos16<ROLE>(a.stream_off, a.stream_base, (size_t)cell, (uint32_t)lane, L.pgrp);
+                else
+                    pos_a[c] = p3_load_pos<ROLE>(a.stream_pos, (size_t)cell, (uint32_t)lane);
+            }
             if (ROLE == 1) st_own_mask[c] = (a.valid_mask + (size_t)cell * 16)[(uint32_t)lane & 15u];
         }
         P3Halo st_halo;
@@ -708,7 +792,7 @@
         }
         m = __builtin_fmaxf(m, p3_commit_halo<CHECK>(st_halo, s_cells, L.halo_lds));
         if (CHECK) p3_check(m, lane, a.inexact);
-        if (ROLE == 1 && !(ablate_flags(a.ablate) & 1)) p3_lf_finish<WORDS, STREAM>(a, lds.hist, lf_item, lf_values);
+        if (ROLE == 1 && !(ablate_flags(a.ablate) & 1)) p3_lf_finish<WORDS, STREAM, P16>(a, lds.hist, lf_item, lf_values);
     }
     if (ROLE == 1) {
         for (uint32_t base = kLfTilesPerPass; base < my_tiles; base += kLfTilesPerPass) {
@@ -717,7 +801,7 @@
             P3LfValues x;
             p3_lf_hop_a(a, walk.first + k * walk.step, k < my_tiles, lf_tid, it);
             p3_lf_hop_b<C16>(a, plane, it, x);
-            if (!(ablate_flags(a.ablate) & 1)) p3_lf_finish<WORDS, STREAM>(a, lds.hist, it, x);
+            if (!(ablate_flags(a.ablate) & 1)) p3_lf_finish<WORDS, STREAM, P16>(a, lds.hist, it, x);
         }
     }
     lds_barrier();
@@ -726,10 +810,10 @@
 
     int it = 0;
     for (uint32_t tile = walk.first; tile < walk.end;) {
-        p3_tile<0, ROLE, CHECK, WORDS, C16, STREAM>(a, plane, lds, it, tile + walk.step < walk.end, min(tile + 2 * walk.step, last), tid, lane, wave, slot_a, L, ga, gb, own_a, own_b, pos_a, pos_b);
+        p3_tile<0, ROLE, CHECK, WORDS, C16, STREAM, P16>(a, plane, lds, it, tile + walk.step < walk.end, min(tile + 2 * walk.step, last), tid, lane, wave, slot_a, L, ga, gb, own_a, own_b, pos_a, pos_b);
         tile += walk.step, it++;
         if (tile >= walk.end) break;
-        p3_tile<1, ROLE, CHECK, WORDS, C16, STREAM>(a, plane, lds, it, tile + walk.step < walk.end, min(tile + 2 * walk.step, last), tid, lane, wave, slot_a, L, ga, gb, own_b, own_a, pos_b, pos_a);
+        p3_tile<1, ROLE, CHECK, WORDS, C16, STREAM, P16>(a, plane, lds, it, tile + walk.step < walk.end, min(tile + 2 * walk.step, last), tid, lane, wave, slot_a, L, ga, gb, own_b, own_a, pos_b, pos_a);
         tile += walk.step, it++;
     }
 }
@@ -755,7 +839,7 @@
     return a;
 }
 
-template <bool CHECK, bool WORDS, bool C16 = false, bool STREAM = false>
+template <bool CHECK, bool WORDS, bool C16 = false, bool STREAM = false, bool P16 = false>
 __global__ void __launch_bounds__(kP3Threads) predict_histogram_kernel3(const PredArgs a0) {
     PredArgs a = pred_plane_view(a0, blockIdx.y);
     if (C16) a.coefs = reinterpret_cast<const int32_t *>(reinterpret_cast<const int16_t *>(a0.coefs) + blockIdx.y * a0.coef_stride);
@@ -774,9 +858,9 @@
         reinterpret_cast<uint32_t *>(s_cells + (i / ((kP3ImageBytes - kP3ZeroOff) / 4)) * kP3ImageBytes + kP3ZeroOff)[i % ((kP3ImageBytes - kP3ZeroOff) / 4)] = 0;
     uint32_t early_poll = 0;
     if (wave & 1)
-        p3_run<1, CHECK, WORDS, C16, STREAM>(a, lds, tid, lane, wave, early_poll);
+        p3_run<1, CHECK, WORDS, C16, STREAM, P16>(a, lds, tid, lane, wave, early_poll);
     else
-        p3_run<0, CHECK, WORDS, C16, STREAM>(a, lds, tid, lane, wave, early_poll);
+        p3_run<0, CHECK, WORDS, C16, STREAM, P16>(a, lds, tid, lane, wave, early_poll);
     lds_barrier();
     trace_stamp(a.trace, blockIdx.x, 13, tid);
     pred_hand_over<CHECK>(a, s_hist, reinterpret_cast<uint32_t *>(s_ring), tid, kP3Threads, early_poll);
@@ -889,9 +973,13 @@
     a.halo_list = p.halo_list;
     a.ablate = p.k2_ablate;
     (void)hipGetLastError();
-    a.stream_pos = b.stream_pos;
-    if (b.stream_pos && !(b.words && b.coefs16)) return hipErrorInvalidValue;
-    if (b.words && b.coefs16 && b.stream_pos)
+    a.stream_pos = b.stream_pos, a.stream_off = b.stream_off, a.stream_base = b.stream_base, a.stream_len = b.stream_len;
+    const bool pos16 = b.stream_off && b.stream_base;
+    if ((b.stream_off || b.stream_base) && (!pos16 || b.stream_pos)) return hipErrorInvalidValue;
+    if ((b.stream_pos || pos16) && !(b.words && b.coefs16)) return hipErrorInvalidValue;
+    if (b.words && b.coefs16 && pos16)
+        hipLaunchKernelGGL((predict_histogram_kernel3<false, true, true, true, true>), dim3(blocks, b.n_planes), dim3(kP3Threads), 0, stream, a);
+    else if (b.words && b.coefs16 && b.stream_pos)
         hipLaunchKernelGGL((predict_histogram_kernel3<false, true, true, true>), dim3(blocks, b.n_planes), dim3(kP3Threads), 0, stream, a);
     else if (b.words && b.coefs16)
         hipLaunchKernelGGL((predict_histogram_kernel3<false, true, true>), dim3(blocks, b.n_planes), dim3(kP3Threads), 0, stream, a);
diff --git a/frave_amd/csrc/kernels.hpp b/frave_amd/csrc/kernels.hpp
--- a/frave_amd/csrc/kernels.hpp
+++ b/frave_amd/csrc/kernels.hpp
@@ -69,6 +69,15 @@
 constexpr uint32_t kFitShards = 16;
 constexpr uint32_t kPredAccRing = 8, kPredAccWords = 16;
 
+constexpr uint32_t kPosGroups = 24;
+constexpr uint32_t pos_group(uint32_t heap) {
+    if (heap >= 64) return 5 + heap / 32;
+    uint32_t g = 0;
+    while (heap) g++, heap >>= 1;
+    return g;
+}
+static_assert(pos_group(0) == 0 && pos_group(1) == 1 && pos_group(3) == 2 && pos_group(63) == 6 && pos_group(64) == 7 && pos_group(511) == 20, "position groups");
+
 struct QMatrix {
     int32_t q[32];
 };
@@ -89,6 +98,9 @@
     const PredictParams *params = nullptr;
     PredictParams pp[3] = {};
     const uint32_t *stream_pos = nullptr;
+    const uint16_t *stream_off = nullptr;
+    const uint32_t *stream_base = nullptr;
+    uint32_t stream_len = 0;
     uint16_t *words = nullptr;
 };
 constexpr int kPredAnyInt32 = 0, kPredPromised = 1, kPredForwardOutput = 2;
diff --git a/include/fri_hip.h b/include/fri_hip.h
--- a/include/fri_hip.h
+++ b/include/fri_hip.h
@@ -125,6 +125,9 @@
                               uint32_t *d_hist, uint64_t *d_n_out_of_alphabet, void *stream);
 
 int fri_hip_plan_set_stream_order(fri_hip_plan *plan, const uint32_t *order, uint64_t n);
+int fri_hip_plan_stream_position_format(const fri_hip_plan *plan);
+int fri_hip_plan_compact_stream_positions(const fri_hip_plan *plan, const uint32_t *order, uint64_t n, uint32_t *base, uint16_t *offset, uint32_t *largest_offset,
+                                          int *format);
 int fri_hip_symbol_stream_batch_dev(fri_hip_plan *plan, uint32_t n_planes, const int32_t *d_coefs, size_t coef_stride, const uint8_t *d_bucket, const int32_t *d_prediction,
                                     size_t out_stride, uint16_t *d_symbols, size_t symbol_stride, void *stream);
 
diff --git a/integration/hip_sys.rs b/integration/hip_sys.rs
--- a/integration/hip_sys.rs
+++ b/integration/hip_sys.rs
@@ -80,6 +80,8 @@
     pub fn fri_hip_predict_image(plan: *mut fri_hip_plan, coefs: *const i32, fit: c_int, value_params: *mut f32, width_params: *mut f32, bucket: *mut u8, prediction: *mut i32, hist: *mut u32, n_out_of_alphabet: *mut u64) -> c_int;
     pub fn fri_hip_predict_image_dev(plan: *mut fri_hip_plan, d_coefs: *const i32, fit: c_int, value_params: *mut f32, width_params: *mut f32, d_bucket: *mut u8, d_prediction: *mut i32, d_hist: *mut u32, d_n_out_of_alphabet: *mut u64, stream: *mut c_void) -> c_int;
     pub fn fri_hip_plan_set_stream_order(plan: *mut fri_hip_plan, order: *const u32, n: u64) -> c_int;
+    pub fn fri_hip_plan_stream_position_format(plan: *const fri_hip_plan) -> c_int;
+    pub fn fri_hip_plan_compact_stream_positions(plan: *const fri_hip_plan, order: *const u32, n: u64, base: *mut u32, offset: *mut u16, largest_offset: *mut u32, format: *mut c_int) -> c_int;
     pub fn fri_hip_symbol_stream_batch_dev(plan: *mut fri_hip_plan, n_planes: u32, d_coefs: *const i32, coef_stride: usize, d_bucket: *const u8, d_prediction: *const i32, out_stride: usize, d_symbols: *mut u16, symbol_stride: usize, stream: *mut c_void) -> c_int;
     pub fn fri_hip_encode_symbols_batch_dev(plan: *mut fri_hip_plan, n_images: u32, d_pixels: *const u8, pixel_stride: usize, qmatrix: *const i32, fit: c_int, d_params: *mut f32, d_coefs: *mut i32, coef_stride: usize, d_node_words: *mut u16, word_stride: usize, d_symbols: *mut u16, symbol_stride: usize, d_hist: *mut u32, d_n_out_of_alphabet: *mut u64, d_fit_out_of_range: *mut u64, stream: *mut c_void) -> c_int;
     pub fn fri_hip_encode_image_symbols(plan: *mut fri_hip_plan, pixels: *const u8, qmatrix: *const i32, fit: c_int, value_params: *mut f32, width_params: *mut f32, symbols: *mut u16, hist: *mut u32, n_out_of_alphabet: *mut u64) -> c_int;
```
